# taylorlu/voicepuppet

Measured on AMD Instinct MI355X. Metric: PixReferNet G+D step frames/sec @256x256 bs=32, higher is better.
Workload: dtype bf16; 1 GPU; PixReferNet G+D training step (G + 3xD + VGG16-conv3_3 perceptual + TF-Adam x2), 256x256, ngf=ndf=64, global batch 32 = 32 per GPU; global_batch=32, per_gpu_batch=32, parallelism=dp1

## Files before the change

include/vp_hip.h:

```cpp
#ifndef VP_HIP_H_
#define VP_HIP_H_

#include <stddef.h>
#include <stdint.h>

#ifdef __cplusplus
extern "C" {
#endif

enum vp_status { VP_OK = 0, VP_ERR_ARG = -1, VP_ERR_HIP = -2, VP_ERR_WORKSPACE = -3, VP_ERR_STATE = -4 };
enum vp_dtype { VP_F32 = 0, VP_BF16 = 1 };
enum vp_act { VP_ACT_NONE = 0, VP_ACT_LRELU = 1, VP_ACT_RELU = 2, VP_ACT_TANH = 3, VP_ACT_SIGMOID = 4, VP_ACT_RELU6 = 5, VP_ACT_LEAKY = 6 };

int vp_version(void);
const char* vp_last_error(void);

typedef struct vp_pixrefer_desc {
  int batch;
  int height;
  int ngf, ndf;
  int dtype;
  int training;
  float l1_weight;
  float gan_weight;
  int per_sample_bn;
  int streams;
  int d_backward_fork;
  int d_beside_vgg;
} vp_pixrefer_desc;

size_t vp_pixrefer_desc_size(void);

typedef struct vp_pixrefer vp_pixrefer_t;

size_t vp_pixrefer_param_count(const vp_pixrefer_desc* d, int which);
int vp_pixrefer_param_info(const vp_pixrefer_desc* d, int which, int index, char* name, int name_cap,
                           size_t* offset, int* ndim, int64_t shape[4]);

size_t vp_pixrefer_workspace_bytes(const vp_pixrefer_desc* d);
int vp_pixrefer_validate_plan(const vp_pixrefer_desc* d);

int vp_pixrefer_create(const vp_pixrefer_desc* d, void* workspace, size_t workspace_bytes,
                       float* params_g, float* params_d, const float* params_vgg,
                       float* grads_g, float* grads_d, void* stream, vp_pixrefer_t** out);
void vp_pixrefer_destroy(vp_pixrefer_t* h);

int vp_pixrefer_params_changed(vp_pixrefer_t* h);
int vp_pixrefer_optimizer_stepped(vp_pixrefer_t* h);

int vp_pixrefer_forward(vp_pixrefer_t* h, const float* inputs, const float* fg_inputs,
                        const float* targets, const float* masks, void* stream);

int vp_pixrefer_forward_fg3(vp_pixrefer_t* h, const float* inputs, const float* fg_inputs3, const float* targets, void* stream);

int vp_pixrefer_backward(vp_pixrefer_t* h, void* stream);
int vp_pixrefer_backward_update(vp_pixrefer_t* h, float* m_g, float* v_g, float* m_d, float* v_d, int step_t_g, int step_t_d,
                                float lr, float beta1, float beta2, float eps, void* stream);

int vp_pixrefer_backward_d(vp_pixrefer_t* h, void* stream);
int vp_pixrefer_backward_g(vp_pixrefer_t* h, void* stream);
int vp_pixrefer_backward_d_fork(vp_pixrefer_t* h, void* stream);
int vp_pixrefer_backward_d_join(vp_pixrefer_t* h, void* stream);
void* vp_pixrefer_side_stream(vp_pixrefer_t* h);
int vp_reserve_streams(void);
void* vp_host_stream(void);
int vp_pixrefer_use_streams(vp_pixrefer_t* h, int n);
int vp_pixrefer_set_option(vp_pixrefer_t* h, const char* key, int value);
long long vp_pixrefer_counter(vp_pixrefer_t* h, const char* key);
int vp_pixrefer_fetch(vp_pixrefer_t* h, int what, void* dst, void* stream);
int vp_pixrefer_backward_g_stages(void);
int vp_pixrefer_backward_g_stage(vp_pixrefer_t* h, int stage, void* stream);
int vp_pixrefer_update_bucket(vp_pixrefer_t* h, int which, int bucket, float* m, float* v, int step_t, float lr, float beta1,
                              float beta2, float eps, void* stream);

int vp_pixrefer_tensor(vp_pixrefer_t* h, const char* name, void** ptr, int64_t shape[4], int* dtype);

int vp_profile_enable(int on);
size_t vp_profile_collect(char* json, size_t cap);

int vp_pixrefer_pack_frames(const unsigned char* example_frames, const unsigned char* current_frames, const int* crops,
                            int n, int img_size, float* inputs, float* fg_inputs, float* targets, float* masks, void* stream);

int vp_tune(const char* key, int value);
int vp_pixrefer_phase_ms(vp_pixrefer_t* h, float* ms, int cap);
float vp_pixrefer_mark_ms(vp_pixrefer_t* h, int from, int to);

int vp_grad_pack_bf16(const float* src, void* dst_bf16, size_t n, void* stream);
int vp_grad_unpack_bf16(const void* src_bf16, float* dst, size_t n, float scale, void* stream);

int vp_adam_tf(float* params, const float* grads, float* m, float* v, size_t n, int step_t,
               float lr, float beta1, float beta2, float eps, void* stream);

typedef struct vp_conv_desc {
  int kind;
  int n, h, w;
  int cin, cout;
  int ksize, stride, pad;
  int dtype;
  int in_act;
  int out_act;
} vp_conv_desc;

size_t vp_conv_workspace_bytes(const vp_conv_desc* d);
int vp_conv_fwd(const vp_conv_desc* d, const void* x, const float* in_scale, const float* in_shift,
                const float* w, const float* bias, void* y, void* workspace, void* stream);
int vp_conv_bwd_data(const vp_conv_desc* d, const void* dy, const float* w, void* dx, void* workspace, void* stream);
size_t vp_conv3x3_c64_bwd_data_pooled_workspace_bytes(const vp_conv_desc* d);
int vp_conv3x3_c64_bwd_data_pooled(const vp_conv_desc* d, const void* dy_pool, const unsigned char* code, const float* w, const void* ref,
                                   void* dx, void* workspace, int fused, void* stream);
int vp_conv_bwd_weight(const vp_conv_desc* d, const void* x, const float* in_scale, const float* in_shift,
                       const void* dy, float* dw, void* workspace, void* stream);

size_t vp_bn_workspace_bytes(int pixels, int c, int dtype);
int vp_bn_stats(const void* y, int pixels, int c, int dtype, const float* gamma, const float* beta, float eps,
                float* scale, float* shift, float* mean, float* rstd, void* workspace, void* stream);
int vp_bn_bwd(const void* y, const void* dz, void* dy, int pixels, int c, int dtype, const float* gamma,
              const float* mean, const float* rstd, float* dgamma, float* dbeta, void* workspace, void* stream);

typedef struct vp_logmel_desc {
  int sample_rate, num_mel_bins, win_length, hop_step, fft_length;
  float lower_hz, upper_hz;
  int batch, samples;
} vp_logmel_desc;
typedef struct vp_logmel vp_logmel_t;
size_t vp_logmel_workspace_bytes(const vp_logmel_desc* d);
int vp_logmel_frames(const vp_logmel_desc* d);
int vp_logmel_create(const vp_logmel_desc* d, void* workspace, size_t workspace_bytes, void* stream, vp_logmel_t** out);
void vp_logmel_destroy(vp_logmel_t* h);
int vp_logmel_forward(vp_logmel_t* h, const float* pcm, float* out, void* stream);

typedef struct vp_bfmnet_desc {
  int batch;
  int frames;
  int num_mel_bins;
  int trunk_dtype;
} vp_bfmnet_desc;
typedef struct vp_bfmnet vp_bfmnet_t;
size_t vp_bfmnet_param_count(void);
int vp_bfmnet_param_info(int index, char* name, int name_cap, size_t* offset, int* ndim, int64_t shape[4]);
size_t vp_bfmnet_workspace_bytes(const vp_bfmnet_desc* d);
int vp_bfmnet_create(const vp_bfmnet_desc* d, void* workspace, size_t workspace_bytes, const float* params,
                     void* stream, vp_bfmnet_t** out);
void vp_bfmnet_destroy(vp_bfmnet_t* h);
int vp_bfmnet_params_changed(vp_bfmnet_t* h);
int vp_bfmnet_forward(vp_bfmnet_t* h, const float* ears, const float* mfccs, const int* seq_len, float* out, void* stream);
int vp_bfmnet_set_decoder_dropout(vp_bfmnet_t* h, const float* mask0, const float* mask1);
int vp_bfmnet_tensor(vp_bfmnet_t* h, const char* name, void** ptr, int64_t shape[4]);

typedef struct vp_bfmstream_desc {
  int struct_bytes;
  int max_chunk_frames;
// ... 217 lines not shown
```

voicepuppet_amd/_lib.py:

```python
import ctypes
import os

_HERE = os.path.dirname(os.path.abspath(__file__))
LIB_PATH = os.environ.get("VP_LIB", os.path.join(_HERE, "libvp_hip.so"))

VP_F32, VP_BF16 = 0, 1
ACT_NONE, ACT_LRELU, ACT_RELU, ACT_TANH, ACT_SIGMOID = 0, 1, 2, 3, 4


class PixReferDesc(ctypes.Structure):
  _fields_ = [("batch", ctypes.c_int), ("height", ctypes.c_int), ("ngf", ctypes.c_int), ("ndf", ctypes.c_int),
              ("dtype", ctypes.c_int), ("training", ctypes.c_int), ("l1_weight", ctypes.c_float),
              ("gan_weight", ctypes.c_float), ("per_sample_bn", ctypes.c_int),
              ("streams", ctypes.c_int), ("d_backward_fork", ctypes.c_int), ("d_beside_vgg", ctypes.c_int)]


class ConvDesc(ctypes.Structure):
  _fields_ = [("kind", ctypes.c_int), ("n", ctypes.c_int), ("h", ctypes.c_int), ("w", ctypes.c_int),
              ("cin", ctypes.c_int), ("cout", ctypes.c_int), ("ksize", ctypes.c_int), ("stride", ctypes.c_int),
              ("pad", ctypes.c_int), ("dtype", ctypes.c_int), ("in_act", ctypes.c_int), ("out_act", ctypes.c_int)]


class LogMelDesc(ctypes.Structure):
  _fields_ = [("sample_rate", ctypes.c_int), ("num_mel_bins", ctypes.c_int), ("win_length", ctypes.c_int),
              ("hop_step", ctypes.c_int), ("fft_length", ctypes.c_int), ("lower_hz", ctypes.c_float),
              ("upper_hz", ctypes.c_float), ("batch", ctypes.c_int), ("samples", ctypes.c_int)]


class BfmNetDesc(ctypes.Structure):
  _fields_ = [("batch", ctypes.c_int), ("frames", ctypes.c_int), ("num_mel_bins", ctypes.c_int), ("trunk_dtype", ctypes.c_int)]


class BfmStreamDesc(ctypes.Structure):
  _fields_ = [("struct_bytes", ctypes.c_int), ("max_chunk_frames", ctypes.c_int), ("num_mel_bins", ctypes.c_int),
              ("trunk_dtype", ctypes.c_int), ("sample_rate", ctypes.c_int), ("lower_hz", ctypes.c_float), ("upper_hz", ctypes.c_float)]


class BfmStreamGroupDesc(ctypes.Structure):
  _fields_ = [("struct_bytes", ctypes.c_int), ("slots", ctypes.c_int), ("max_chunk_frames", ctypes.c_int), ("num_mel_bins", ctypes.c_int),
              ("trunk_dtype", ctypes.c_int), ("sample_rate", ctypes.c_int), ("lower_hz", ctypes.c_float), ("upper_hz", ctypes.c_float)]


BFMSTREAM_GROUP_MAX_SLOTS = 128


class PuppetDesc(ctypes.Structure):
  _fields_ = [("struct_bytes", ctypes.c_int), ("slots", ctypes.c_int), ("frame_batch", ctypes.c_int), ("img_size", ctypes.c_int),
              ("face_size", ctypes.c_int)]


PUPPET_MAX_SLOTS = 128


class JpegDesc(ctypes.Structure):
  _fields_ = [("struct_bytes", ctypes.c_uint32), ("max_frames", ctypes.c_int32), ("height", ctypes.c_int32), ("width", ctypes.c_int32),
              ("quality", ctypes.c_int32)]


class PcmInDesc(ctypes.Structure):
  _fields_ = [("struct_bytes", ctypes.c_int), ("slots", ctypes.c_int), ("out_rate", ctypes.c_int), ("max_in_frames", ctypes.c_int),
              ("n_rates", ctypes.c_int), ("rates", ctypes.c_int * 8)]


PCMIN_MAX_SLOTS, PCMIN_MAX_CHANNELS = 128, 8
PCM_S16, PCM_F32 = 0, 1


class BfmModel(ctypes.Structure):
  _fields_ = [("nver", ctypes.c_int), ("ntri", ctypes.c_int), ("meanshape", ctypes.c_void_p), ("idBase", ctypes.c_void_p),
              ("exBase", ctypes.c_void_p), ("meantex", ctypes.c_void_p), ("texBase", ctypes.c_void_p), ("tri", ctypes.c_void_p),
              ("point_buf", ctypes.c_void_p), ("center", ctypes.c_double * 3), ("focal", ctypes.c_double),
              ("image_center", ctypes.c_double), ("sh", ctypes.c_double * 5)]


_P = ctypes.c_void_p
_SIGNATURES = {
    "vp_version": (ctypes.c_int, []),
    "vp_last_error": (ctypes.c_char_p, []),
    "vp_pixrefer_param_count": (ctypes.c_size_t, [ctypes.POINTER(PixReferDesc), ctypes.c_int]),
    "vp_pixrefer_param_info": (ctypes.c_int, [ctypes.POINTER(PixReferDesc), ctypes.c_int, ctypes.c_int, ctypes.c_char_p,
                                              ctypes.c_int, ctypes.POINTER(ctypes.c_size_t), ctypes.POINTER(ctypes.c_int),
                                              ctypes.POINTER(ctypes.c_int64)]),
    "vp_pixrefer_workspace_bytes": (ctypes.c_size_t, [ctypes.POINTER(PixReferDesc)]),
    "vp_pixrefer_validate_plan": (ctypes.c_int, [ctypes.POINTER(PixReferDesc)]),
    "vp_pixrefer_create": (ctypes.c_int, [ctypes.POINTER(PixReferDesc), _P, ctypes.c_size_t, _P, _P, _P, _P, _P, _P,
                                          ctypes.POINTER(_P)]),
    "vp_pixrefer_destroy": (None, [_P]),
    "vp_pixrefer_params_changed": (ctypes.c_int, [_P]),
    "vp_pixrefer_optimizer_stepped": (ctypes.c_int, [_P]),
    "vp_pixrefer_forward": (ctypes.c_int, [_P, _P, _P, _P, _P, _P]),
    "vp_pixrefer_forward_fg3": (ctypes.c_int, [_P, _P, _P, _P, _P]),
    "vp_pixrefer_desc_size": (ctypes.c_size_t, []),
    "vp_pixrefer_backward": (ctypes.c_int, [_P, _P]),
    "vp_pixrefer_backward_update": (ctypes.c_int, [_P, _P, _P, _P, _P, ctypes.c_int, ctypes.c_int, ctypes.c_float, ctypes.c_float,
                                                   ctypes.c_float, ctypes.c_float, _P]),
    "vp_pixrefer_backward_d": (ctypes.c_int, [_P, _P]),
    "vp_pixrefer_backward_g": (ctypes.c_int, [_P, _P]),
    "vp_pixrefer_backward_d_fork": (ctypes.c_int, [_P, _P]),
    "vp_pixrefer_backward_d_join": (ctypes.c_int, [_P, _P]),
    "vp_pixrefer_backward_g_stages": (ctypes.c_int, []),
    "vp_pixrefer_backward_g_stage": (ctypes.c_int, [_P, ctypes.c_int, _P]),
    "vp_pixrefer_side_stream": (ctypes.c_void_p, [_P]),
    "vp_pixrefer_use_streams": (ctypes.c_int, [_P, ctypes.c_int]),
    "vp_pixrefer_set_option": (ctypes.c_int, [_P, ctypes.c_char_p, ctypes.c_int]),
    "vp_pixrefer_fetch": (ctypes.c_int, [_P, ctypes.c_int, _P, _P]),
    "vp_pixrefer_counter": (ctypes.c_longlong, [_P, ctypes.c_char_p]),
    "vp_crc32c": (ctypes.c_uint, [_P, ctypes.c_size_t, ctypes.c_uint]),
    "vp_pixrefer_phase_ms": (ctypes.c_int, [_P, ctypes.POINTER(ctypes.c_float), ctypes.c_int]),
    "vp_grad_pack_bf16": (ctypes.c_int, [_P, _P, ctypes.c_size_t, _P]),
    "vp_grad_unpack_bf16": (ctypes.c_int, [_P, _P, ctypes.c_size_t, ctypes.c_float, _P]),
    "vp_pixrefer_update_bucket": (ctypes.c_int, [_P, ctypes.c_int, ctypes.c_int, _P, _P, ctypes.c_int, ctypes.c_float, ctypes.c_float, ctypes.c_float,
                                                 ctypes.c_float, _P]),
    "vp_resize_paste_workspace_bytes": (ctypes.c_size_t, [ctypes.c_int, ctypes.c_int]),
    "vp_resize_paste_u8": (ctypes.c_int, [_P, ctypes.c_int, ctypes.c_int, ctypes.c_int, ctypes.c_int, ctypes.c_int, ctypes.c_int, _P, ctypes.c_int,
                                          ctypes.c_int, ctypes.c_int, ctypes.c_int, _P, _P]),
    "vp_resize_linear_table": (ctypes.c_int, [ctypes.c_int, ctypes.c_int, ctypes.c_int, _P, _P, _P, _P]),
    "vp_mm_workspace_bytes": (ctypes.c_size_t, [ctypes.c_int, ctypes.c_int, ctypes.c_int]),
    "vp_mm_fwd_f32": (ctypes.c_int, [_P, ctypes.c_int, _P, ctypes.c_int, ctypes.c_int, _P, _P, ctypes.c_int, ctypes.c_int, ctypes.c_int, ctypes.c_int, _P, _P]),
    "vp_mm_bwd_data_f32": (ctypes.c_int, [_P, ctypes.c_int, _P, ctypes.c_int, ctypes.c_int, _P, ctypes.c_int, ctypes.c_int, ctypes.c_int, ctypes.c_int,
                                          ctypes.c_int, _P, _P]),
    "vp_mm_bwd_weight_f32": (ctypes.c_int, [_P, ctypes.c_int, _P, ctypes.c_int, _P, ctypes.c_int, ctypes.c_int, ctypes.c_int, ctypes.c_int, _P, _P]),
    "vp_mm_packed_bytes": (ctypes.c_size_t, [ctypes.c_int, ctypes.c_int, ctypes.c_int, ctypes.c_int]),
    "vp_mm_pack_desc_bytes": (ctypes.c_size_t, []),
    "vp_mm_pack_desc": (ctypes.c_int, [ctypes.c_size_t, ctypes.c_int, ctypes.c_int, ctypes.c_int, ctypes.c_int, ctypes.c_int, ctypes.c_int, ctypes.c_size_t, _P]),
    "vp_mm_pack_table": (ctypes.c_int, [_P, ctypes.c_int, _P, _P, _P]),
    "vp_mm_fwd_f32_packed": (ctypes.c_int, [_P, ctypes.c_int, _P, _P, _P, ctypes.c_int, ctypes.c_int, ctypes.c_int, ctypes.c_int, _P, _P]),
    "vp_mm_bwd_data_f32_packed": (ctypes.c_int, [_P, ctypes.c_int, _P, _P, ctypes.c_int, ctypes.c_int, ctypes.c_int, ctypes.c_int, ctypes.c_int, _P, _P]),
    "vp_pixrefer_mark_ms": (ctypes.c_float, [_P, ctypes.c_int, ctypes.c_int]),
    "vp_profile_enable": (ctypes.c_int, [ctypes.c_int]),
    "vp_tune": (ctypes.c_int, [ctypes.c_char_p, ctypes.c_int]),
    "vp_reserve_streams": (ctypes.c_int, []),
    "vp_host_stream": (ctypes.c_void_p, []),
    "vp_pixrefer_pack_frames": (ctypes.c_int, [_P, _P, _P, ctypes.c_int, ctypes.c_int, _P, _P, _P, _P, _P]),
    "vp_profile_collect": (ctypes.c_size_t, [ctypes.c_char_p, ctypes.c_size_t]),
    "vp_pixrefer_tensor": (ctypes.c_int, [_P, ctypes.c_char_p, ctypes.POINTER(_P), ctypes.POINTER(ctypes.c_int64),
                                          ctypes.POINTER(ctypes.c_int)]),
    "vp_adam_tf": (ctypes.c_int, [_P, _P, _P, _P, ctypes.c_size_t, ctypes.c_int, ctypes.c_float, ctypes.c_float,
                                  ctypes.c_float, ctypes.c_float, _P]),
    "vp_conv_workspace_bytes": (ctypes.c_size_t, [ctypes.POINTER(ConvDesc)]),
    "vp_conv_fwd": (ctypes.c_int, [ctypes.POINTER(ConvDesc), _P, _P, _P, _P, _P, _P, _P, _P]),
    "vp_conv_bwd_data": (ctypes.c_int, [ctypes.POINTER(ConvDesc), _P, _P, _P, _P, _P]),
    "vp_conv_bwd_weight": (ctypes.c_int, [ctypes.POINTER(ConvDesc), _P, _P, _P, _P, _P, _P, _P]),
    "vp_conv3x3_c64_bwd_data_pooled_workspace_bytes": (ctypes.c_size_t, [ctypes.POINTER(ConvDesc)]),
    "vp_conv3x3_c64_bwd_data_pooled": (ctypes.c_int, [ctypes.POINTER(ConvDesc), _P, _P, _P, _P, _P, _P, ctypes.c_int, _P]),
    "vp_bn_workspace_bytes": (ctypes.c_size_t, [ctypes.c_int, ctypes.c_int, ctypes.c_int]),
    "vp_bn_stats": (ctypes.c_int, [_P, ctypes.c_int, ctypes.c_int, ctypes.c_int, _P, _P, ctypes.c_float, _P, _P, _P, _P, _P, _P]),
    "vp_logmel_workspace_bytes": (ctypes.c_size_t, [ctypes.POINTER(LogMelDesc)]),
    "vp_logmel_frames": (ctypes.c_int, [ctypes.POINTER(LogMelDesc)]),
    "vp_logmel_create": (ctypes.c_int, [ctypes.POINTER(LogMelDesc), _P, ctypes.c_size_t, _P, ctypes.POINTER(_P)]),
    "vp_logmel_destroy": (None, [_P]),
    "vp_logmel_forward": (ctypes.c_int, [_P, _P, _P, _P]),
    "vp_bfmnet_param_count": (ctypes.c_size_t, []),
    "vp_bfmnet_param_info": (ctypes.c_int, [ctypes.c_int, ctypes.c_char_p, ctypes.c_int, ctypes.POINTER(ctypes.c_size_t),
                                            ctypes.POINTER(ctypes.c_int), ctypes.POINTER(ctypes.c_int64)]),
    "vp_bfmnet_workspace_bytes": (ctypes.c_size_t, [ctypes.POINTER(BfmNetDesc)]),
    "vp_bfmnet_create": (ctypes.c_int, [ctypes.POINTER(BfmNetDesc), _P, ctypes.c_size_t, _P, _P, ctypes.POINTER(_P)]),
    "vp_bfmnet_destroy": (None, [_P]),
    "vp_bfmnet_params_changed": (ctypes.c_int, [_P]),
    "vp_bfmnet_forward": (ctypes.c_int, [_P, _P, _P, _P, _P, _P]),
    "vp_bfmnet_set_decoder_dropout": (ctypes.c_int, [_P, _P, _P]),
    "vp_bfmnet_tensor": (ctypes.c_int, [_P, ctypes.c_char_p, ctypes.POINTER(_P), ctypes.POINTER(ctypes.c_int64)]),
    "vp_bfmstream_desc_size": (ctypes.c_size_t, []),
    "vp_bfmstream_context": (ctypes.c_int, [ctypes.POINTER(BfmStreamDesc)] + [ctypes.POINTER(ctypes.c_int)] * 5),
    "vp_bfmstream_frames_after": (ctypes.c_longlong, [ctypes.POINTER(BfmStreamDesc), ctypes.c_longlong, ctypes.c_int]),
    "vp_bfmstream_workspace_bytes": (ctypes.c_size_t, [ctypes.POINTER(BfmStreamDesc)]),
    "vp_bfmstream_create": (ctypes.c_int, [ctypes.POINTER(BfmStreamDesc), _P, ctypes.c_size_t, _P, _P, ctypes.POINTER(_P)]),
    "vp_bfmstream_destroy": (None, [_P]),
    "vp_bfmstream_params_changed": (ctypes.c_int, [_P]),
    "vp_bfmstream_reset": (ctypes.c_int, [_P, _P]),
    "vp_bfmstream_ready": (ctypes.c_int, [_P, ctypes.c_longlong]),
    "vp_bfmstream_ready_finish": (ctypes.c_int, [_P]),
    "vp_bfmstream_push": (ctypes.c_int, [_P, _P, ctypes.c_longlong, _P, _P, _P]),
    "vp_bfmstream_finish": (ctypes.c_int, [_P, _P, _P, _P]),
    "vp_bfmstream_tensor": (ctypes.c_int, [_P, ctypes.c_char_p, ctypes.POINTER(_P), ctypes.POINTER(ctypes.c_int64)]),
    "vp_bfmstream_group_desc_size": (ctypes.c_size_t, []),
    "vp_puppet_desc_size": (ctypes.c_size_t, []),
    "vp_puppet_workspace_bytes": (ctypes.c_size_t, [ctypes.POINTER(PuppetDesc)]),
    "vp_puppet_create": (ctypes.c_int, [ctypes.POINTER(PuppetDesc), _P, ctypes.c_size_t, _P, ctypes.POINTER(_P)]),
    "vp_puppet_destroy": (None, [_P]),
    "vp_puppet_attach": (ctypes.c_int, [_P, ctypes.c_int, _P, _P, _P, ctypes.c_int, ctypes.c_int, ctypes.c_int, _P]),
    "vp_puppet_set_backgrounds": (ctypes.c_int, [_P, _P, ctypes.c_int]),
    "vp_puppet_splice": (ctypes.c_int, [_P, _P, ctypes.c_int, _P, ctypes.c_int, _P, _P]),
    "vp_puppet_condition": (ctypes.c_int, [_P, _P, ctypes.c_int, _P, ctypes.c_int, _P, _P, _P, _P]),
    "vp_puppet_tensor": (ctypes.c_int, [_P, ctypes.c_char_p, ctypes.POINTER(_P), ctypes.POINTER(ctypes.c_int64)]),
    "vp_puppet_slot_info": (ctypes.c_int, [_P, ctypes.c_int, ctypes.POINTER(ctypes.c_int)]),
    "vp_jpeg_desc_size": (ctypes.c_size_t, []),
    "vp_jpeg_workspace_bytes": (ctypes.c_size_t, [ctypes.POINTER(JpegDesc)]),
    "vp_jpeg_frame_capacity": (ctypes.c_size_t, [ctypes.POINTER(JpegDesc)]),
    "vp_jpeg_create": (ctypes.c_int, [ctypes.POINTER(JpegDesc), _P, ctypes.c_size_t, _P, ctypes.POINTER(_P)]),
# ... 134 lines not shown
```

voicepuppet_amd/csrc/conv_ops.h:

```cpp
#pragma once
#include <stdlib.h>
#include <string.h>

#include "launch.h"

namespace vp {

struct ConvGeomX : ConvGeom {
  int CoutT;
};

inline ConvGeomX make_geom(int kind, int ks, int stride, int pad, int N, int Hin, int Win, int Cin, int Cin_real, int Cout) {
  ConvGeomX g;
  g.kind = kind; g.ks = ks; g.stride = stride; g.pad = pad;
  g.N = N; g.Hin = Hin; g.Win = Win;
  if (kind == 0) { g.Hout = (Hin + 2 * pad - ks) / stride + 1; g.Wout = (Win + 2 * pad - ks) / stride + 1; }
  else { g.Hout = 2 * Hin; g.Wout = 2 * Win; }
  g.Cin = Cin; g.Cin_real = Cin_real; g.Cout = Cout;
  g.CoutT = Cout < 8 ? 8 : Cout;
  return g;
}

inline int kc_elems(int is_bf16) { return is_bf16 ? 32 : 16; }

// ... 10 lines not shown
    if (rows % 128 == 0) return 0;
    if (rows % 64 == 0) return 1;
    if (rows <= 16) return 2;
    return rows > 64 ? 0 : 1;
  }
  if (rows <= 64) return 5;
  return P > 16 ? 3 : 4;
}

constexpr int IGEMM_SPLITK_TARGET_DEFAULT = 64;
inline int& igemm_splitk_target_knob() { static int v = IGEMM_SPLITK_TARGET_DEFAULT; return v; }
inline int pick_igemm_splitk(int blocks, int nchunk) {
  const int target = igemm_splitk_target_knob();
  const int cap = plan_misc_knob(1);
  const int minchunk = plan_misc_knob(2);
  if (blocks >= 256 || blocks >= target) return 1;
  int s = (target + blocks - 1) / blocks;
  if (s > nchunk / minchunk) s = nchunk / minchunk;
  if (s > cap) s = cap;
  return s < 1 ? 1 : s;
}

inline void set_single_src(PixSrc& x, const void* p, int C, const float* a, const float* b, int act, int group_n) {
  x.ptr[0] = p; x.ptr[1] = nullptr; x.C[0] = C; x.C[1] = 0;
  x.aff_a[0] = a; x.aff_b[0] = b; x.aff_a[1] = nullptr; x.aff_b[1] = nullptr;
  x.act = act; x.group_n = group_n > 0 ? group_n : (1 << 30);
}

struct LaunchForm {
  bool bias = false, ref = false, xa_lrelu = false, xa_relu = false, x_affine = false;
  bool stats = false;
  int x_act = 0, ref_act = 0;
};

struct IgemmPlan {
  IgemmArgs a;
  int cfg;
  LaunchForm form;
  PackDesc pack;
  size_t pack_elems;
  size_t partial_bytes;
};

struct IgemmPin { int cfg, splitk; };

inline void finish_igemm(IgemmPlan& p, int rows, int is_bf16, const IgemmPin* pin = nullptr) {
  IgemmArgs& a = p.a;
  const int P = a.N * a.Hg * a.Wg;
  a.Kpad = round_up(a.ntaps * a.Cin, kc_elems(is_bf16));
  p.cfg = pick_igemm_cfg(rows, P, a.Kpad);
  if (!is_bf16 && a.ntaps == 1 && p.cfg == 0) {
    const long long b128 = (long long)((P + 127) / 128) * (rows / 128), b64 = 2 * b128;
    if (((b64 + 255) / 256) * 64 < ((b128 + 255) / 256) * 128) p.cfg = 1;
  }
  if (pin) p.cfg = pin->cfg;
  int bc, bp;
  igemm_tile(p.cfg, &bc, &bp);
  a.CoutPad = round_up(rows, bc);
  if (a.ntaps == 1) { a.log2Cin = 30; a.cin_mask = 0x3fffffff; }
  else { a.log2Cin = ilog2(a.Cin); a.cin_mask = a.Cin - 1; }
  const int blocks = ((P + bp - 1) / bp) * (a.CoutPad / bc) * a.nclass;
  a.splitk = pin ? pin->splitk : pick_igemm_splitk(blocks, a.Kpad / kc_elems(is_bf16));
  p.partial_bytes = a.splitk > 1 ? (size_t)a.nclass * a.splitk * P * a.CoutPad * sizeof(float) : 0;
  {
    const bool tc4 = p.cfg == 0 || p.cfg == 1 || p.cfg == 6 || p.cfg == 7 || p.cfg == 8 || p.cfg == 9;
    a.rowperm = (tc4 && rows % 64 == 0) ? 1 : 0;
    p.pack.perm = a.rowperm;
  }
  a.wp_rows = round_up(rows, 128);
  p.pack.rows_pad = a.wp_rows;
  p.pack.Kpad = a.Kpad;
  p.pack.kc = kc_elems(is_bf16);
  p.pack_elems = (size_t)a.nclass * a.wp_rows * a.Kpad;
}

inline int& patch_tiles_knob() { static int v = 7; return v; }
inline int& patch_small_knob() { static int v = 3; return v; }
inline int& patch_longk_knob() { static int v = 1; return v; }
inline int& patch3_knob() { static int v = 1; return v; }
inline int& wgrad_big_knob() { static int v = 1; return v; }
inline int& patch4_knob() { static int v = 1; return v; }
inline int& c64_knob() { static int v = 1; return v; }
inline int& pool_bwd_fused_knob() { static int v = 1; return v; }
inline int& cout1_knob() { static int v = 256; return v; }
inline int& wgrad1_rows_knob() { static int v = 512; return v; }
inline int& dc64_knob() { static int v = 1; return v; }
inline int& s2c64_knob() { static int v = 512; return v; }
inline int& s2c64_pair_knob() { static int v = 1; return v; }
constexpr int PATCH_MIN_BLOCKS_DEFAULT = 192;
inline int& patch_minblk_knob() { static int v = PATCH_MIN_BLOCKS_DEFAULT; return v; }

inline void patch_tile_hw(int bp, int* th, int* tw) { *th = bp == 128 ? 8 : 16; *tw = bp == 512 ? 32 : 16; }
inline int patch_tile_pixels(int bc) {
  const int k = patch_small_knob();
  if (bc == 256) return (k & 2) ? 128 : 256;
  return (k & 1) ? 256 : 512;
}

inline int patch_tile_rows(int rows, int on) {
  if ((on & 1) && rows % 256 == 0) return 256;
  if ((on & 2) && rows % 128 == 0) return 128;
  if ((on & 4) && rows % 64 == 0) return 64;
  return 0;
}

inline bool plan_patch_eligible(const IgemmPlan& p, int rows, int is_bf16, bool single_src, bool any_grid = false) {
  const int on = patch_tiles_knob();
  const int minblk = any_grid ? 0 : patch_minblk_knob();
  const IgemmArgs& a = p.a;
  const int kc = kc_elems(is_bf16);
  if (!on || !single_src || a.nclass != 1 || a.sh != 1 || a.sw != 1 || a.os != 1 || a.ntaps < 9 || a.Cin % kc || a.Cin < kc) return false;
  if (rows % 64 || a.Cout % 8 || a.ldY % 8 || a.Hg < 16 || a.Wg < 16 || a.Hof != a.Hg || a.Wof != a.Wg) return false;
  const bool p4 = patch4_knob() && is_bf16 && a.ntaps == 16 && rows % 128 == 0;
  if (!p4 && patch_longk_knob() && rows >= 512 && rows % 256 == 0 && a.ntaps * a.Cin >= 4096 && (long long)a.N * a.Hg * a.Wg >= 256 * 256) return false;
  const int bc = p4 ? 128 : patch_tile_rows(rows, on);
  if (!bc) return false;
  int th, tw;
  patch_tile_hw(p4 ? 256 : patch_tile_pixels(bc), &th, &tw);
  const long long blocks = (long long)a.N * ((a.Hg + th - 1) / th) * ((a.Wg + tw - 1) / tw) * (rows / bc);
  const long long p4min = (long long)a.ntaps * a.Cin >= 8192 ? 256 : 512;
  if (p4 && !any_grid && patch_minblk_knob() > 1) {
    if (blocks < p4min) return false;
  } else if (blocks < minblk) return false;
  if ((size_t)a.N * a.Hin * a.Win * a.Cin * (is_bf16 ? 2 : 4) >= 0x70000000ull) return false;
  int ks = 0;
  while (ks * ks < a.ntaps) ++ks;
  if (ks * ks != a.ntaps) return false;
  const int sh = a.taps[0].dh[ks] - a.taps[0].dh[0], sw = a.taps[0].dw[1] - a.taps[0].dw[0];
  if ((sh != 1 && sh != -1) || (sw != 1 && sw != -1)) return false;
  for (int t = 0; t < a.ntaps; ++t)
    if (a.taps[0].dh[t] != a.taps[0].dh[0] + (t / ks) * sh || a.taps[0].dw[t] != a.taps[0].dw[0] + (t % ks) * sw) return false;
  return true;
}
inline void plan_make_patch(IgemmPlan& p, int rows, int is_bf16) {
  IgemmArgs& a = p.a;
  const bool p4 = patch4_knob() && is_bf16 && a.ntaps == 16 && rows % 128 == 0;
  const int bc = p4 ? 128 : patch_tile_rows(rows, patch_tiles_knob());
  int ks = 0;
  while (ks * ks < a.ntaps) ++ks;
  a.kern = CK_PATCH; a.p_kw = ks;
  a.p_dhf = a.taps[0].dh[0]; a.p_dwf = a.taps[0].dw[0];
  a.p_dhs = a.taps[0].dh[ks] - a.taps[0].dh[0]; a.p_dws = a.taps[0].dw[1] - a.taps[0].dw[0];
  const int bp = p4 ? 256 : patch_tile_pixels(bc);
  p.cfg = bc == 256 ? (bp == 128 ? 15 : 10) : (bc == 128 ? (bp == 256 ? 13 : 11) : (bp == 256 ? 14 : 12));
  a.CoutPad = round_up(rows, bc);
  a.splitk = 1;
  p.partial_bytes = 0;
  a.rowperm = 1;
  p.pack.perm = 1;
  p.pack.kswap = 1;
}

inline int& patch_xcd_knob() { static int v = 0; return v; }
inline int& patch2_knob() { static int v = 1; return v; }
inline bool plan_patch2_eligible(const IgemmPlan& p, int rows, int is_bf16, int c0, int c1) {
  const IgemmArgs& a = p.a;
  const int kc = kc_elems(is_bf16);
  if (!patch2_knob() || a.nclass != 4 || a.ntaps != 4 || a.os != 2 || a.sh != 1 || a.sw != 1) return false;
  if (c0 + c1 != a.Cin || c0 % (2 * kc) || c1 % (2 * kc) || c0 < 2 * kc) return false;
  if (rows % 64 || rows > 128 || a.Cout % 8 || a.ldY % 8 || a.Hg < 16 || a.Wg < 16 || a.Hof != 2 * a.Hg || a.Wof != 2 * a.Wg) return false;
  const long long blocks = (long long)a.N * ((a.Hg + 15) / 16) * ((a.Wg + 15) / 16) * 4;
  if (blocks < patch_minblk_knob()) return false;
  const size_t cmax = c0 > c1 ? c0 : c1;
  if ((size_t)a.N * a.Hin * a.Win * cmax * (is_bf16 ? 2 : 4) >= 0x70000000ull) return false;
  for (int cls = 0; cls < 4; ++cls)
    for (int t = 0; t < 4; ++t)
// ... 281 lines not shown
```

voicepuppet_amd/csrc/launch.h:

```cpp
#pragma once
#include <hip/hip_runtime.h>

#include "conv_args.h"
#include "pointwise_args.h"

namespace vp {

hipError_t launch_igemm(const IgemmArgs& a, int is_bf16, int cfg, hipStream_t st);
void igemm_tile(int cfg, int* bc, int* bp);
hipError_t launch_igemm_patch(const IgemmArgs& a, int is_bf16, int bc, int bp, hipStream_t st);
bool patch3_eligible(const IgemmArgs& a, int is_bf16);
hipError_t launch_igemm_patch3(const IgemmArgs& a, int is_bf16, int bc, int bp, hipStream_t st);
bool patch4_eligible(const IgemmArgs& a, int is_bf16);
hipError_t launch_igemm_patch4(const IgemmArgs& a, hipStream_t st);
bool conv_cin8_eligible(const IgemmArgs& a, int is_bf16);
bool conv_cout8_eligible(const IgemmArgs& a, int is_bf16);
bool conv_dcout8_eligible(const IgemmArgs& a, int is_bf16);
bool conv_cout4_eligible(const IgemmArgs& a, int is_bf16);
bool conv_kernel_ok(const IgemmArgs& a, int is_bf16);
const char* conv_kernel_name(int kern);
bool conv_c64_eligible(const IgemmArgs& a, int is_bf16);
hipError_t launch_conv_c64(const IgemmArgs& a, hipStream_t st);
bool conv_dc64_eligible(const IgemmArgs& a, int is_bf16);
hipError_t launch_conv_dc64(const IgemmArgs& a, hipStream_t st);
int conv_dc64_grid(const IgemmArgs& a);
bool conv_dc256_eligible(const IgemmArgs& a, int is_bf16);
int conv_dc256_grid(const IgemmArgs& a);
hipError_t launch_conv_dc256(const IgemmArgs& a, hipStream_t st);
bool conv_s2c64_eligible(const IgemmArgs& a, int is_bf16);
int conv_s2c64_grid(const IgemmArgs& a);
int conv_s2c64_tiles_per_image(const IgemmArgs& a);
hipError_t launch_conv_s2c64(const IgemmArgs& a, hipStream_t st);
bool conv_cout1_bwd_eligible(const Cout1Args& a);
hipError_t launch_conv_cout1_bwd(const Cout1Args& a, hipStream_t st);
bool conv_cout1_wgrad_eligible(const Cout1Args& a);
hipError_t launch_conv_cout1_wgrad(const Cout1Args& a, hipStream_t st);
hipError_t launch_cout1_wgrad_prof(const Cout1Args& a, hipStream_t st);
hipError_t launch_cout1_bwd_prof(const Cout1Args& a, hipStream_t st);
hipError_t launch_igemm_patch2(const IgemmArgs& a, int is_bf16, int bc, int bp, hipStream_t st);
hipError_t launch_igemm_smallp(const IgemmArgs& a, int is_bf16, hipStream_t st);
struct SmallPArgs;
hipError_t launch_smallp(const SmallPArgs& s, int is_bf16, hipStream_t st);
hipError_t launch_smallp_fused(const SmallPArgs& s, int is_bf16, hipStream_t st);
hipError_t launch_wgrad(const WgradArgs& a, int is_bf16, int cfg, hipStream_t st);
bool wgrad_mm_eligible(const WgradArgs& a, int cfg);
hipError_t launch_wgrad_mm(const WgradArgs& a, int cfg, hipStream_t st);
hipError_t launch_wgrad_tr(const WgradArgs& a, hipStream_t st, const char** variant = nullptr, int* tile_cols = nullptr);
void wgrad_tile(int cfg, int* bm, int* bn);

void profile_enable(int on);
void profile_tag(const char* tag);
size_t profile_collect(char* out, size_t cap);

hipError_t launch_pack_weights(const PackDesc* d_descs, int ndesc, const float* master, void* packed, int is_bf16, hipStream_t st);
hipError_t launch_pack_weights_one(const PackDesc& d, const float* master, void* packed, int is_bf16, hipStream_t st);
int bn_nchunk(int Pg, int C, int G, int is_bf16);
hipError_t launch_bn_stats(const BnArgs& a, int is_bf16, hipStream_t st);
hipError_t launch_bn_finalize(const BnArgs& a, hipStream_t st);
bool bn_small(const BnArgs& a);
hipError_t launch_bn_small_fwd(const BnArgs& a, void* out_lrelu, void* out_relu, int is_bf16, hipStream_t st);
hipError_t launch_bn_small_bwd(const BnArgs& a, int is_bf16, hipStream_t st);
hipError_t launch_bn_bwd(const BnArgs& a, int is_bf16, hipStream_t st);
hipError_t launch_bn_bwd_tail(const BnArgs& a, int is_bf16, hipStream_t st);
hipError_t launch_colsum(const BnArgs& a, int creal, float* out, int accumulate, int is_bf16, hipStream_t st);
hipError_t launch_colsum_tail(const BnArgs& a, int creal, float* out, int accumulate, hipStream_t st);
hipError_t launch_act_apply(const void* y, const float* sc, const float* sh, int C, int Pg, size_t npix,
                            void* out_lrelu, void* out_relu, int is_bf16, hipStream_t st);
hipError_t launch_tap_gather(const TapArgs& a, hipStream_t st);
hipError_t launch_tap_spread(const TapArgs& a, int is_bf16, hipStream_t st);
hipError_t launch_frame_pack(const FramePackArgs& a, hipStream_t st);
hipError_t launch_pack_inputs(const PackInputsArgs& a, int is_bf16, hipStream_t st);
int composite_nblocks(int N, int HW);
hipError_t launch_composite_fwd(const CompositeArgs& a, int is_bf16, hipStream_t st);
hipError_t launch_composite_bwd(const CompositeArgs& a, int is_bf16, hipStream_t st);
hipError_t launch_gan_loss(const GanLossArgs& a, int is_bf16, hipStream_t st);
int perceptual_nblocks(size_t half, int is_bf16);
hipError_t launch_perceptual(const PerceptualArgs& a, int is_bf16, hipStream_t st);
hipError_t launch_loss_final(const LossFinalArgs& a, hipStream_t st);
hipError_t launch_maxpool_fwd(const void* x, void* y, int B, int H, int W, int C, int is_bf16, hipStream_t st);
hipError_t launch_maxpool_bwd(const void* x, const void* dy, void* dx, int B, int H, int W, int C, int is_bf16, hipStream_t st);
hipError_t launch_maxpool_bwd_code(const void* code, const void* dy, void* dx, int B, int H, int W, int C, int is_bf16, hipStream_t st);
hipError_t launch_relu_bwd(const void* y, void* d, size_t n, int is_bf16, hipStream_t st);
hipError_t launch_adam(const AdamArgs& a, hipStream_t st);
hipError_t launch_fetch(const FetchArgs& a, hipStream_t st);
hipError_t launch_grad_pack_bf16(const float* src, void* dst, size_t n, hipStream_t st);
hipError_t launch_grad_unpack_bf16(const void* src, float* dst, size_t n, float scale, hipStream_t st);

struct ConvGeom {
  int kind;
  int ks, stride, pad;
  int N, Hin, Win, Hout, Wout;
  int Cin, Cin_real;
  int Cout;
};

inline int ilog2(int v) { int l = 0; while ((1 << l) < v) ++l; return l; }
inline int round_up(int v, int m) { return (v + m - 1) / m * m; }

}
```

voicepuppet_amd/csrc/ops_api.hip:

```cpp
#include <string.h>

#include <string>

#include "conv_ops.h"
#include "errors.h"
#include "audio_args.h"
#include "launch.h"
#include "vp_common.h"

using namespace vp;

namespace {

bool conv_desc_ok(const vp_conv_desc* d) {
  if (!d || d->n < 1 || d->h < 1 || d->w < 1) return false;
  if (d->cin < 8 || (d->cin & (d->cin - 1))) return false;
  if (d->kind == 1 && (d->ksize != 4 || d->stride != 2 || d->pad != 1)) return false;
  if (d->kind != 0 && d->kind != 1) return false;
  if (d->ksize < 1 || d->ksize > 4 || d->stride < 1 || d->stride > 2) return false;
  if (d->kind == 0 && d->stride == 2 && (d->ksize != 4 || d->pad != 1 || (d->h & 1) || (d->w & 1))) return false;
  return d->dtype == VP_F32 || d->dtype == VP_BF16;
}

ConvGeomX geom_of(const vp_conv_desc* d) {
  return make_geom(d->kind, d->ksize, d->stride, d->pad, d->n, d->h, d->w, d->cin, d->cin, d->cout);
}

size_t align256(size_t v) { return (v + 255) & ~(size_t)255; }

const void* zero_page(char* ws, size_t used, hipStream_t st) {
  char* z = ws + align256(used);
  (void)hipMemsetAsync(z, 0, 256, st);
  return z;
}

}

extern "C" {

int vp_pixrefer_pack_frames(const unsigned char* example_frames, const unsigned char* current_frames, const int* crops,
                            int n, int img_size, float* inputs, float* fg_inputs, float* targets, float* masks, void* stream) {
  if (!example_frames || !current_frames || !crops || !inputs || !fg_inputs || !targets || !masks || n < 1 || img_size < 2) {
    set_err("vp_pixrefer_pack_frames: bad argument");
    return VP_ERR_ARG;
  }
  FramePackArgs a;
  a.ex = example_frames; a.cur = current_frames; a.crops = crops;
  a.inputs = inputs; a.fg_inputs = fg_inputs; a.targets = targets; a.masks = masks;
  a.N = n; a.S = img_size;
  VP_HIP_CHECK(launch_frame_pack(a, (hipStream_t)stream));
  return VP_OK;
}

extern "C" void vp_phase_marks_enable(int on);

int vp_tune(const char* key, int value) {
  if (!key) return VP_ERR_ARG;
  const std::string k(key);
  if (k == "patch_tiles") { patch_tiles_knob() = value; return VP_OK; }
  if (k == "patch_min_blocks") { patch_minblk_knob() = value < 0 ? PATCH_MIN_BLOCKS_DEFAULT : value; return VP_OK; }
  if (k == "patch_small_tiles") { patch_small_knob() = value; return VP_OK; }
  if (k == "patch_long_k_on_256") { patch_longk_knob() = value; return VP_OK; }
  if (k == "wgrad_tr") { wgrad_tr_knob() = value; return VP_OK; }
  if (k == "patch3") { patch3_knob() = value; return VP_OK; }
  if (k == "c64") { c64_knob() = value; return VP_OK; }
  if (k == "dc64") { dc64_knob() = value; return VP_OK; }
  if (k == "pool_bwd_fused") { pool_bwd_fused_knob() = value < 0 || value > 4 ? 1 : value; return VP_OK; }
  if (k == "cout1_wgrad_rows" && value > 0) { wgrad1_rows_knob() = value; return VP_OK; }
  if (k == "cout1_bwd") { cout1_knob() = value < 0 ? 256 : value; return VP_OK; }
  if (k == "s2c64") { s2c64_knob() = value; return VP_OK; }
  if (k == "wgrad_big") { wgrad_big_knob() = value; return VP_OK; }
  if (k == "patch4") { patch4_knob() = value; return VP_OK; }
  if (k == "s2c64_pair") { s2c64_pair_knob() = value; return VP_OK; }
  if (k == "bfm_dwproj") { bfm_dwproj_knob() = value; return VP_OK; }
  if (k == "patch2") { patch2_knob() = value; return VP_OK; }
  if (k == "patch_xcd") { patch_xcd_knob() = value; return VP_OK; }
  if (k == "smallp_max_pixels") { smallp_knob() = value; return VP_OK; }
  if (k == "igemm_splitk_target") { igemm_splitk_target_knob() = value < 0 ? IGEMM_SPLITK_TARGET_DEFAULT : value; return VP_OK; }
  if (k == "wgrad_fixed_x10") { wgrad_cost_knob(0) = value; return VP_OK; }
  if (k == "wgrad_slab_tile_x1000") { wgrad_cost_knob(2) = value < 0 ? 150 : value; return VP_OK; }
  if (k == "wgrad_slab_x100") { wgrad_cost_knob(1) = value; return VP_OK; }
  if (k == "smallp_split_target") { plan_misc_knob(0) = value; return VP_OK; }
  if (k == "igemm_splitk_cap") { plan_misc_knob(1) = value; return VP_OK; }
  if (k == "igemm_splitk_minchunk") { plan_misc_knob(2) = value; return VP_OK; }
  if (k == "wgrad_resident_blocks") { plan_misc_knob(3) = value; return VP_OK; }
  if (k == "igemm_small_grid") { igemm_small_grid_knob() = value; return VP_OK; }
  if (k == "thin_blocks_cout8" && value > 0) { thin_blocks_knob(0) = value; return VP_OK; }
  if (k == "thin_blocks_dcout8" && value > 0) { thin_blocks_knob(1) = value; return VP_OK; }
  if (k == "thin_blocks_cout4" && value > 0) { thin_blocks_knob(2) = value; return VP_OK; }
  if (k == "thin_blocks_cin8" && value > 0) { thin_blocks_knob(3) = value; return VP_OK; }
  if (k == "phase_marks") { vp_phase_marks_enable(value); return VP_OK; }
  set_err("vp_tune: unknown key %s", key);
  return VP_ERR_ARG;
}

static unsigned* smallp_counter_page(char* ws, size_t used, const IgemmArgs& a, hipStream_t st) {
  unsigned* c = (unsigned*)(ws + align256(used) + 256);
  (void)hipMemsetAsync(c, 0, (size_t)smallp_counters(a) * sizeof(unsigned), st);
  return c;
}

size_t vp_conv_workspace_bytes(const vp_conv_desc* d) {
  if (!conv_desc_ok(d)) return 0;
  const int bf = d->dtype == VP_BF16, es = bf ? 2 : 4;
  const ConvGeomX g = geom_of(d);
  size_t best = 0;
  {
    IgemmPlan p = plan_fwd(g, 0, bf);
    best = align256(p.pack_elems * es) + p.partial_bytes;
    plan_kernel(p, g.Cout, bf, d->cin, 0, FAM_SMALLP, LaunchForm{});
    if (p.a.kern == CK_SMALLP) {
      const size_t b = align256(p.pack_elems * es) + align256(p.partial_bytes) + 512 + (size_t)smallp_counters(p.a) * sizeof(unsigned);
      if (b > best) best = b;
    }
  }
  if ((d->cout & (d->cout - 1)) == 0 && d->cout >= 8) {
    IgemmPlan p = plan_bwd_data(g, 0, 0, d->cin, d->cin, d->cin, bf);
    size_t b = align256(p.pack_elems * es) + p.partial_bytes;
    if (b > best) best = b;
    plan_kernel(p, d->cin, bf, d->cout, 0, FAM_SMALLP, LaunchForm{});
    if (p.a.kern == CK_SMALLP) {
      b = align256(p.pack_elems * es) + align256(p.partial_bytes) + 512 + (size_t)smallp_counters(p.a) * sizeof(unsigned);
      if (b > best) best = b;
    }
    for (int plain = 0; plain < 2; ++plain) {
      WgradPlan w = plan_wgrad(g, bf, plain != 0);
      if (w.partial_bytes + 512 > best) best = w.partial_bytes + 512;
    }
  }
  return best + 1024;
}

int vp_conv_fwd(const vp_conv_desc* d, const void* x, const float* in_scale, const float* in_shift,
                const float* w, const float* bias, void* y, void* workspace, void* stream) {
  if (!conv_desc_ok(d) || !x || !w || !y || !workspace) { set_err("vp_conv_fwd: bad argument"); return VP_ERR_ARG; }
  const int bf = d->dtype == VP_BF16, es = bf ? 2 : 4;
  hipStream_t st = (hipStream_t)stream;
  const ConvGeomX g = geom_of(d);
  IgemmPlan p = plan_fwd(g, 0, bf);
  p.a.out_act = d->out_act;
  LaunchForm f;
  f.bias = bias != nullptr; f.x_affine = in_scale != nullptr; f.x_act = d->in_act;
  const bool plain = d->in_act == ACT_NONE && !in_scale;
  plan_kernel(p, g.Cout, bf, d->cin, 0, plain ? (FAM_SMALLP | FAM_PATCH | FAM_PATCH2 | (d->out_act == ACT_NONE ? FAM_S2C64 : 0)) : 0, f);
  char* ws = (char*)workspace;
  VP_HIP_CHECK(launch_pack_weights_one(p.pack, w, ws, bf, st));
  IgemmArgs a = p.a;
  set_single_src(a.x, x, d->cin, in_scale, in_shift, d->in_act, 0);
  a.Wp = ws;
  a.partial = (float*)(ws + align256(p.pack_elems * es));
// ... 276 lines not shown
```

voicepuppet_amd/csrc/plan_pixrefer.hip:

```cpp
#include <math.h>
#include <stdio.h>
#include <string.h>

#include <mutex>
#include <string>
#include <utility>
#include <vector>

#include "conv_ops.h"
#include "errors.h"
#include "launch.h"
#include "smallp_args.h"
#include "vp_common.h"

namespace vp {

thread_local char g_err[512] = "";
void set_err(const char* fmt, ...) {
  va_list ap;
  va_start(ap, fmt);
  vsnprintf(g_err, sizeof(g_err), fmt, ap);
  va_end(ap);
}

struct Arena {
  char* base;
  size_t off, cap;
  std::vector<std::pair<size_t, size_t>>* track = nullptr;
  void* alloc(size_t bytes) {
    off = (off + 255) & ~(size_t)255;
    void* p = base ? base + off : nullptr;
    if (track) track->push_back({off, bytes});
    off += bytes;
    return p;
  }
};

struct BnBuf {
  float *a, *b, *mu, *rstd, *c1, *c2, *c1g, *c2g;
  double *pb, *pbg;
};

struct Tens {
  std::string name;
  void* y = nullptr;
  void* dz = nullptr;
  int N = 0, H = 0, W = 0, C = 0;
  bool is_f32 = false;
  bool has_bn = false;
  bool is_input = false;
  bool dz_written = false;
  void* dz2 = nullptr;
  bool dz2_written = false;
  void* xa[3] = {nullptr, nullptr, nullptr};
  bool need_act[3] = {false, false, false};
  BnBuf bn{};
  int producer = -1;
  int n_bwd_consumers = 0;
  int dz_writes = 0;
  bool bn_bwd_done = false;
  bool hi = false;
  void* dz32 = nullptr;
  double* cs_part = nullptr;
  int cs_chunks = 0;
  int pb_cap = 0, pbg_cap = 0;
  int bst_chunks = 0, bst_chunks_g = 0;
  size_t elems() const { return (size_t)N * H * W * C; }
};

struct Layer {
  std::string scope;
  ConvGeomX g;
  int src[2] = {-1, -1};
  int nsrc = 1;
  int in_act = ACT_NONE;
  int out_act = ACT_NONE;
  int out = -1;
  bool has_bn = false;
  size_t w_off = 0, b_off = 0, gamma_off = 0, beta_off = 0;
  size_t pk_fwd = 0, pk_bwd[2] = {0, 0}, pk_bwd_alt[2] = {0, 0};
  bool need_bwd[2] = {false, false};
  IgemmPlan fwd, bwd[2], bwd_alt[2];
  IgemmPlan bwd_pair;
  size_t pk_bwd_pair = 0;
  bool has_pair = false;
  IgemmPlan fwd_half;
  size_t pk_fwd_half = 0;
  bool has_fwd_half = false;
  WgradPlan wg;
  size_t desc0 = 0, desc1 = 0;
  bool tapgemm = false;
  bool fwd_stats = false;
  float* tap_S = nullptr;
  void* tap_dyS = nullptr;
  unsigned* sp_cnt_fwd = nullptr;
  unsigned* sp_cnt_bwd[2] = {nullptr, nullptr};
  unsigned* sp_cnt_pair = nullptr;
};

struct ParamInfo { std::string name; size_t off; int ndim; int64_t shape[4]; };

struct Net {
  std::vector<Tens> t;
  std::vector<Layer> l;
  std::vector<ParamInfo> manifest;
  size_t nparams = 0;
  int batch = 0, groups = 1;
  float* params = nullptr;
  float* grads = nullptr;
  char* packed = nullptr;
  size_t packed_elems = 0;
  std::vector<PackDesc> descs;
  PackDesc* d_descs = nullptr;
  unsigned* sp_cnt = nullptr;
  size_t sp_cnt_n = 0;
};

}

using namespace vp;

struct vp_pixrefer {
  vp_pixrefer_desc d;
  int bf16, es;
  Net G, D, V;
  void *gin, *gfg, *din, *vin;
  float *y4, *o4, *outputs, *outputs_fg, *logits, *predict, *losses;
  void *dl_d, *dl_g, *d_din, *d_vin, *dy4, *df3;
  void *vpool1, *vpool2, *d_vpool1, *d_vpool2;
  unsigned char* vpool_code[2];
  bool pool_codes_written;
  bool pool_fuse_ok[2];
  bool pool_bwd_fused;
  bool pool_dz_stale[2];
  double *comp_partial, *perc_partial, *bn_partial;
  char* scratch;
  char* scratch2;
  double* bn_partial2;
  char* scratch3;
  double* bn_partial3;
  char* scratch4;
  double* bn_partial4;
  hipStream_t side, branch;
  hipStream_t branch2;
  hipEvent_t ev_b2join;
  bool use_b2;
  hipEvent_t ev_fork, ev_join, ev_bfork, ev_bjoin;
  hipEvent_t ev_upd_b, ev_upd_m;
  bool overlap, forked;
  int bst_count;
  int bst_on;
  int vgg_fork_layer;
  bool store_first_raw;
  bool ov_on;
  int dfork_point;
  bool dsplit_on;
  hipEvent_t mark[64];
  int nmark;
  bool marks_made;
  int dfork_pending;
  void* zeros;
  size_t scratch_bytes;
  int n_comp, n_perc;
  struct { bool active, d_done; float *m_g, *v_g, *m_d, *v_d; float lr_t_g, lr_t_d, beta1, beta2, eps; } upd;
  int upd_mask;
  bool params_dirty;
  bool vgg_dirty;
  const float *in_targets, *in_masks;
};

namespace vp {

static int add_tensor(Net& n, const std::string& name, int N, int H, int W, int C, bool has_bn, bool is_input) {
  Tens t;
  t.name = name; t.N = N; t.H = H; t.W = W; t.C = C; t.has_bn = has_bn; t.is_input = is_input;
  n.t.push_back(t);
  return (int)n.t.size() - 1;
}

static void add_param(Net& n, const std::string& name, std::initializer_list<int64_t> shape, size_t* off_out) {
  ParamInfo p;
  p.name = name; p.off = n.nparams; p.ndim = (int)shape.size();
  size_t cnt = 1;
  int i = 0;
  for (auto s : shape) { p.shape[i++] = s; cnt *= (size_t)s; }
  for (; i < 4; ++i) p.shape[i] = 1;
  *off_out = n.nparams;
  n.nparams += cnt;
  n.manifest.push_back(p);
}

static int add_layer(Net& n, const std::string& prefix, const std::string& scope, int kind, int ks, int stride, int pad,
                     std::initializer_list<int> srcs, int cin_real, int cout, bool has_bn, int in_act, int out_act,
                     const char* wname, const char* bname) {
  Layer L;
  L.scope = scope;
// ... 176 lines not shown
            take(L.bwd_alt[s]);
            L.pk_bwd_alt[s] = L.bwd_alt[s].pack.dst_off;
          } else {
            L.bwd_alt[s].pack.dst_off = L.pk_bwd[s];
            if (L.bwd_alt[s].partial_bytes > *scratch_max) *scratch_max = L.bwd_alt[s].partial_bytes;
          }
        }
      }
      row0 += rows;
    }
    {
      const int s0 = conv_staging(L.bwd[0].a.kern);
      if (L.nsrc == 2 && n.groups == 1 && alt_batch == 0 && L.need_bwd[0] && L.need_bwd[1] && c0 == c1 && !n.t[L.src[0]].is_input &&
          !n.t[L.src[1]].is_input && s0 == conv_staging(L.bwd[1].a.kern) && (s0 == CK_IGEMM || s0 == CK_SMALLP) &&
          L.g.Cin_real == c0 + c1 && c0 % 32 == 0) {
        L.bwd_pair = plan_bwd_data(L.g, L.w_off, 0, c0 + c1, c0 + c1, c0, bf16);
        L.bwd_pair.a.split_c = c0;
        LaunchForm f;
        f.ref = true; f.ref_act = L.in_act;
        const unsigned fams = s0 == CK_SMALLP ? FAM_SMALLP : (s2c64_pair_knob() && L.in_act == ACT_RELU ? FAM_S2C64 : 0);
        plan_kernel(L.bwd_pair, c0 + c1, bf16, L.g.CoutT, 0, fams, f);
        if (s0 != CK_SMALLP || L.bwd_pair.a.kern == CK_SMALLP) {
          take(L.bwd_pair);
          L.pk_bwd_pair = L.bwd_pair.pack.dst_off;
          L.has_pair = true;
        }
      }
    }
    if (want_wgrad) {
      if (L.tapgemm) {
        ConvGeomX gw = make_geom(0, 1, 1, 0, L.g.N, L.g.Hin, L.g.Win, 16, 16, L.g.Cin);
        L.wg = plan_wgrad(gw, bf16);
      } else {
        L.wg = plan_wgrad(L.g, bf16);
      }
      if (L.wg.partial_bytes > *scratch_max) *scratch_max = L.wg.partial_bytes;
    }
  }
  n.packed_elems = pk;
  {
    for (Tens& t : n.t) t.hi = bf16 && t.has_bn && n.groups == 1 && alt_batch == 0 && t.producer >= 0 && n.l[t.producer].fwd.a.kern == CK_SMALLP;
    if (training)
      for (Layer& L : n.l)
        for (int s = 0; s < L.nsrc; ++s)
          if (L.need_bwd[s] && L.bwd[s].a.kern != CK_SMALLP) n.t[L.src[s]].hi = false;
    for (Layer& L : n.l)
      for (int s = 0; s < L.nsrc; ++s)
        if (L.in_act == ACT_NONE) n.t[L.src[s]].hi = false;
  }
  for (Tens& t : n.t) t.pb_cap = t.pbg_cap = 0;
  if (training)
    for (Layer& L : n.l) {
      auto cap = [&](Tens& t, const IgemmPlan& p, int batch, int groups, int& c) {
        if (!t.has_bn || t.hi) return;
        const int k = epi_stat_chunks(p, batch, groups);
        if (k > 0 && k <= BST_MAX_CHUNKS && k > c) c = k;
      };
      for (int s = 0; s < L.nsrc; ++s) {
        if (!L.need_bwd[s]) continue;
        Tens& ts = n.t[L.src[s]];
        cap(ts, L.bwd[s], n.batch, n.groups, ts.pb_cap);
        if (alt_batch > 0) cap(ts, L.bwd_alt[s], alt_batch, 1, ts.pbg_cap);
        if (L.has_pair) cap(ts, L.bwd_pair, n.batch, n.groups, ts.pb_cap);
        if (L.tapgemm && bf16 && ts.has_bn && !ts.hi && L.g.ks == 4 && L.g.stride == 1 && L.g.Cin == 512) {
          if (ts.pb_cap < 256) ts.pb_cap = 256;
          if (alt_batch > 0 && ts.pbg_cap < 256) ts.pbg_cap = 256;
        }
      }
    }
  for (size_t i = 0; i < n.l.size(); ++i) n.l[i].desc1 = i + 1 < n.l.size() ? n.l[i + 1].desc0 : n.descs.size();
  for (Tens& t : n.t) t.n_bwd_consumers = 0;
  n.sp_cnt_n = 0;
  for (Layer& L : n.l) {
    if (L.fwd.a.kern == CK_SMALLP) n.sp_cnt_n += smallp_counters(L.fwd.a);
    for (int s = 0; s < L.nsrc && training; ++s) {
      if (!L.need_bwd[s]) continue;
      n.t[L.src[s]].n_bwd_consumers++;
      if (L.bwd[s].a.kern == CK_SMALLP) n.sp_cnt_n += smallp_counters(L.bwd[s].a);
    }
    if (training && L.has_pair && L.bwd_pair.a.kern == CK_SMALLP) n.sp_cnt_n += smallp_counters(L.bwd_pair.a);
  }
}

static void carve_net(Net& n, Arena& ar, int es, bool training) {
  for (Tens& t : n.t) {
    if (t.name == "decoder_1" || t.name == "layer_5") {
      continue;
    }
    if (!t.is_input) t.y = ar.alloc(t.elems() * (t.hi ? sizeof(float) : (size_t)es));
    for (int k = 1; k < 3; ++k) if (t.need_act[k]) t.xa[k] = ar.alloc(t.elems() * es);
    if (t.has_bn) {
      const size_t gc = (size_t)n.groups * t.C * sizeof(float);
      t.bn.a = (float*)ar.alloc(gc); t.bn.b = (float*)ar.alloc(gc);
      t.bn.mu = (float*)ar.alloc(gc); t.bn.rstd = (float*)ar.alloc(gc);
      t.bn.c1 = (float*)ar.alloc(gc); t.bn.c2 = (float*)ar.alloc(gc);
      t.bn.c1g = (float*)ar.alloc(gc); t.bn.c2g = (float*)ar.alloc(gc);
      t.bn.pb = (training && t.pb_cap) ? (double*)ar.alloc((size_t)n.groups * t.pb_cap * 2 * t.C * sizeof(double)) : nullptr;
      t.bn.pbg = (training && t.pbg_cap) ? (double*)ar.alloc((size_t)t.pbg_cap * 2 * t.C * sizeof(double)) : nullptr;
    }
  }
  for (Layer& L : n.l) {
    if (!L.tapgemm) continue;
    const size_t q = (size_t)L.g.N * L.g.Hin * L.g.Win * 16;
    L.tap_S = (float*)ar.alloc(q * sizeof(float));
    L.tap_dyS = ar.alloc(q * es);
  }
  n.packed = (char*)ar.alloc(n.packed_elems * es);
  n.d_descs = (PackDesc*)ar.alloc(n.descs.size() * sizeof(PackDesc));
  n.sp_cnt = (unsigned*)ar.alloc((n.sp_cnt_n + 1) * sizeof(unsigned));
  {
    unsigned* c = n.sp_cnt;
    for (Layer& L : n.l) {
      if (L.fwd.a.kern == CK_SMALLP) { L.sp_cnt_fwd = c; c += c ? smallp_counters(L.fwd.a) : 0; }
      for (int s = 0; s < L.nsrc && training; ++s)
        if (L.need_bwd[s] && L.bwd[s].a.kern == CK_SMALLP) { L.sp_cnt_bwd[s] = c; c += c ? smallp_counters(L.bwd[s].a) : 0; }
      if (training && L.has_pair && L.bwd_pair.a.kern == CK_SMALLP) { L.sp_cnt_pair = c; c += c ? smallp_counters(L.bwd_pair.a) : 0; }
    }
  }
}

static size_t carve_all(vp_pixrefer* h, char* base, size_t cap, std::vector<std::pair<size_t, size_t>>* track = nullptr) {
  Arena ar{base, 0, cap};
  ar.track = track;
  const vp_pixrefer_desc& d = h->d;
  const int N = d.batch, H = d.height, es = h->es;
  const size_t px = (size_t)N * H * H;
  h->gin = ar.alloc(px * 8 * es);
  h->gfg = ar.alloc(px * 8 * es);
  h->y4 = (float*)ar.alloc(px * 4 * sizeof(float));
  h->o4 = (float*)ar.alloc(px * 4 * sizeof(float));
  h->outputs = (float*)ar.alloc(px * 3 * sizeof(float));
  h->outputs_fg = (float*)ar.alloc(px * 3 * sizeof(float));
  h->losses = (float*)ar.alloc(8 * sizeof(float));
  h->G.t[0].y = h->gin; h->G.t[1].y = h->gfg;
  carve_net(h->G, ar, es, d.training);
  if (d.training) {
    const int hd = H / 8 - 2;
    const size_t M = (size_t)N * hd * hd;
    h->din = ar.alloc(3 * px * 8 * es);
    h->vin = ar.alloc(2 * px * 8 * es);
    h->logits = (float*)ar.alloc(3 * M * sizeof(float));
    h->predict = (float*)ar.alloc(2 * M * sizeof(float));
    h->dl_d = ar.alloc(3 * M * 8 * es);
    h->dl_g = ar.alloc(M * 8 * es);
    h->d_din = ar.alloc(px * 8 * es);
    h->d_vin = ar.alloc(px * 8 * es);
    h->dy4 = ar.alloc(px * 8 * es);
    h->D.t[0].y = h->din; h->V.t[0].y = h->vin;
    carve_net(h->D, ar, es, true);
    carve_net(h->V, ar, es, true);
    for (Tens& t : h->G.t) if (!t.is_input && t.name != "decoder_1") { t.dz = ar.alloc(t.elems() * es); if (t.hi) t.dz32 = ar.alloc(t.elems() * sizeof(float)); }
    for (Tens& t : h->D.t) if (!t.is_input && t.name != "layer_5") { t.dz = ar.alloc(t.elems() * es); t.dz2 = ar.alloc(t.elems() / 3 * es); }
    for (Net* n : {&h->G, &h->D})
      for (Tens& t : n->t) if (h->bf16 && !t.is_input && !t.has_bn && t.C == 64) t.cs_part = (double*)ar.alloc((size_t)512 * 2 * 64 * sizeof(double));
    for (Tens& t : h->V.t) if (!t.is_input) t.dz = ar.alloc(t.elems() / 2 * es);
    for (const Tens& t : h->V.t) {
      if (t.name == "pool1") h->vpool_code[0] = (unsigned char*)ar.alloc(t.elems() / 2);
      if (t.name == "pool2") h->vpool_code[1] = (unsigned char*)ar.alloc(t.elems() / 2);
    }
    h->n_comp = composite_nblocks(N, H * H);
    h->n_perc = perceptual_nblocks((size_t)N * (H / 4) * (H / 4) * 256, h->bf16);
    h->comp_partial = (double*)ar.alloc((size_t)h->n_comp * 2 * sizeof(double));
    h->perc_partial = (double*)ar.alloc((size_t)h->n_perc * sizeof(double));
  }
  h->zeros = ar.alloc(256);
  h->bn_partial = (double*)ar.alloc((size_t)1024 * 2 * 512 * sizeof(double));
  h->scratch = (char*)ar.alloc(h->scratch_bytes);
  if (d.training) {
    h->bn_partial2 = (double*)ar.alloc((size_t)1024 * 2 * 512 * sizeof(double));
    h->scratch2 = (char*)ar.alloc(h->scratch_bytes);
    h->bn_partial3 = (double*)ar.alloc((size_t)1024 * 2 * 512 * sizeof(double));
    h->scratch3 = (char*)ar.alloc(h->scratch_bytes);
    h->bn_partial4 = (double*)ar.alloc((size_t)1024 * 2 * 512 * sizeof(double));
    h->scratch4 = (char*)ar.alloc(h->scratch_bytes);
  }
  return ar.off + 256;
}

static IgemmArgs pool_fused_view(const IgemmPlan& p) {
  static unsigned char set[16] = {};
  IgemmArgs v = launch_view(p, p.form);
  v.pool_code = set;
  v.pool_src = 1;
  return v;
}

static void init_handle(vp_pixrefer* h, const vp_pixrefer_desc* d) {
  h->d = *d;
  h->bf16 = d->dtype == VP_BF16;
  h->es = h->bf16 ? 2 : 4;
  build_generator(h->G, d->batch, d->height, d->ngf, (!d->training && d->per_sample_bn) ? d->batch : 1);
  size_t smax = 0;
  plan_net(h->G, h->bf16, d->training, d->training, 0, &smax);
  if (d->training) {
    build_discriminator(h->D, d->batch, d->height, d->ndf);
    plan_net(h->D, h->bf16, true, true, d->batch, &smax);
    build_vgg(h->V, d->batch, d->height);
    for (Layer& L : h->V.l) L.g.N = 2 * d->batch;
    plan_net(h->V, h->bf16, true, false, d->batch, &smax, true);
    for (const Layer& L : h->V.l) {
      if (L.scope != "conv1/conv1_2" && L.scope != "conv2/conv2_2") continue;
      const int k = L.scope == "conv2/conv2_2", knob = pool_bwd_fused_knob();
      const IgemmArgs& ba = L.bwd_alt[0].a;
      const bool big = !k || (long long)ba.N * (ba.Hg / 4) * (ba.Wg / 16) >= 4096;
      h->pool_fuse_ok[k] = ((knob == 1 && big) || knob == 2 + k || knob == 4) && h->bf16 && conv_kernel_ok(pool_fused_view(L.bwd_alt[0]), h->bf16);
    }
  }
  h->scratch_bytes = smax + 256;
  h->params_dirty = true;
  h->vgg_dirty = true;
}

static bool valid_desc(const vp_pixrefer_desc* d) {
  if (!d) { set_err("pixrefer descriptor: null"); return false; }
  if (d->batch < 1 || d->height < 256 || d->height % 256 != 0) { set_err("pixrefer descriptor: batch %d / height %d (height must be a multiple of 256)", d->batch, d->height); return false; }
  if (d->ngf < 8 || (d->ngf & (d->ngf - 1)) || d->ndf < 8 || (d->ndf & (d->ndf - 1))) { set_err("pixrefer descriptor: ngf %d / ndf %d must be powers of two >= 8", d->ngf, d->ndf); return false; }
  if (d->ngf > 64 || d->ndf > 64) { set_err("pixrefer descriptor: ngf %d / ndf %d > 64 exceed the batch-norm workspace (512 channels)", d->ngf, d->ndf); return false; }
  if (!d->training && d->per_sample_bn && d->batch > 1024) { set_err("pixrefer descriptor: per-sample batch-norm supports at most 1024 frames per call (got %d)", d->batch); return false; }
  if (d->dtype != VP_F32 && d->dtype != VP_BF16) { set_err("pixrefer descriptor: dtype %d", d->dtype); return false; }
  if ((d->streams != 0 && d->streams != 1 && d->streams != 3 && d->streams != 4) || d->d_backward_fork < 0 || d->d_backward_fork > 3 || d->d_beside_vgg < 0 ||
      d->d_beside_vgg > 2) {
    set_err("pixrefer descriptor: schedule fields streams %d / d_backward_fork %d / d_beside_vgg %d", d->streams, d->d_backward_fork, d->d_beside_vgg);
    return false;
  }
  return true;
}

static void fill_src(const Net& n, const Layer& L, PixSrc& x, int group_n, int sample0, int group0, int es) {
  for (int s = 0; s < 2; ++s) {
    x.ptr[s] = nullptr; x.C[s] = 0; x.aff_a[s] = nullptr; x.aff_b[s] = nullptr;
  }
  for (int s = 0; s < L.nsrc; ++s) {
    const Tens& t = n.t[L.src[s]];
    const void* base = (L.in_act != ACT_NONE) ? t.xa[L.in_act] : t.y;
    x.ptr[s] = (const char*)base + (size_t)sample0 * t.H * t.W * t.C * es;
    x.C[s] = t.C;
  }
  x.act = ACT_NONE;
  x.group_n = group_n;
  (void)group0;
}

static int run_pack(vp_pixrefer* h, Net& n, hipStream_t st) {
  if (n.descs.empty()) return VP_OK;
  VP_HIP_CHECK(launch_pack_weights(n.d_descs, (int)n.descs.size(), n.params, n.packed, h->bf16, st));
  return VP_OK;
}

static char* scratch_of(vp_pixrefer* h, int ss) { return ss == 3 ? h->scratch4 : ss == 2 ? h->scratch3 : ss == 1 ? h->scratch2 : h->scratch; }
static double* bnp_of(vp_pixrefer* h, int ss) { return ss == 3 ? h->bn_partial4 : ss == 2 ? h->bn_partial3 : ss == 1 ? h->bn_partial2 : h->bn_partial; }

static int run_bn_stats(vp_pixrefer* h, Net& n, Layer& L, int fused_chunks, hipStream_t st, int ss = 0) {
  Tens& t = n.t[L.out];
  BnArgs b;
  memset(&b, 0, sizeof(b));
  b.y = t.y; b.C = t.C; b.G = n.groups; b.Pg = (n.batch / n.groups) * t.H * t.W;
  b.nchunk = bn_nchunk(b.Pg, b.C, b.G, h->bf16);
  b.partial = bnp_of(h, ss);
  b.gamma = n.params + L.gamma_off; b.beta = n.params + L.beta_off;
  b.aff_a = t.bn.a; b.aff_b = t.bn.b; b.mu = t.bn.mu; b.rstd = t.bn.rstd;
  b.eps = 1e-5f;
  if (fused_chunks > 0) { b.nchunk = fused_chunks; VP_HIP_CHECK(launch_bn_finalize(b, st)); return VP_OK; }
  if (bn_small(b)) {
    VP_HIP_CHECK(launch_bn_small_fwd(b, t.xa[ACT_LRELU], t.xa[ACT_RELU], h->bf16, st));
    return 1;
  }
  VP_HIP_CHECK(launch_bn_stats(b, h->bf16, st));
  return VP_OK;
}

static bool plan_can_pool(const IgemmPlan& p) {
  if (conv_staging(p.a.kern) != CK_PATCH || (p.a.Hg & 1) || (p.a.Wg & 1)) return false;
  int bc, bp;
  igemm_tile(p.cfg, &bc, &bp);
  int th, tw;
  patch_tile_hw(bp, &th, &tw);
  return tw == 16 && th % 2 == 0;
}

// ... 418 lines not shown
  if (!valid_desc(d)) return 0;
  vp_pixrefer tmp{};
  Net* n = manifest_net(d, which, &tmp);
  return n ? n->nparams : 0;
}

int vp_pixrefer_param_info(const vp_pixrefer_desc* d, int which, int index, char* name, int name_cap,
                           size_t* offset, int* ndim, int64_t shape[4]) {
  if (!valid_desc(d)) return VP_ERR_ARG;
  vp_pixrefer tmp{};
  Net* n = manifest_net(d, which, &tmp);
  if (!n || index < 0 || index >= (int)n->manifest.size()) return VP_ERR_ARG;
  const ParamInfo& p = n->manifest[index];
  if (name && name_cap > 0) { strncpy(name, p.name.c_str(), name_cap - 1); name[name_cap - 1] = 0; }
  if (offset) *offset = p.off;
  if (ndim) *ndim = p.ndim;
  if (shape) for (int i = 0; i < 4; ++i) shape[i] = p.shape[i];
  return VP_OK;
}

size_t vp_pixrefer_workspace_bytes(const vp_pixrefer_desc* d) {
  if (!valid_desc(d)) return 0;
  vp_pixrefer* h = new vp_pixrefer{};
  init_handle(h, d);
  const size_t n = carve_all(h, nullptr, 0);
  delete h;
  return n;
}

int vp_pixrefer_validate_plan(const vp_pixrefer_desc* d) {
  if (!valid_desc(d)) return VP_ERR_ARG;
  vp_pixrefer* h = new vp_pixrefer{};
  init_handle(h, d);
  const size_t need = carve_all(h, nullptr, 0);
  std::vector<std::pair<size_t, size_t>> regs;
  char* const base = reinterpret_cast<char*>((uintptr_t)1 << 40);
  carve_all(h, base, need, &regs);
  int rc = VP_OK;
  auto fail = [&](const char* fmt, auto... args) { if (rc == VP_OK) { set_err(fmt, args...); rc = VP_ERR_STATE; } };
  size_t prev_end = 0;
  for (size_t i = 0; i < regs.size(); ++i) {
    if (regs[i].first % 256) fail("region %zu at %zu: not 256-byte aligned", i, regs[i].first);
    if (regs[i].first < prev_end) fail("region %zu at %zu overlaps the previous one (ends %zu)", i, regs[i].first, prev_end);
    prev_end = regs[i].first + regs[i].second;
  }
  if (prev_end + 256 > need + 256 || prev_end > need) fail("carved %zu bytes of a %zu-byte workspace", prev_end, need);
  auto region_of = [&](const void* p, size_t bytes, const char* what) {
    if (!p) { fail("%s: null", what); return; }
    const size_t off = (size_t)((const char*)p - base);
    for (const auto& r : regs)
      if (off >= r.first && off + bytes <= r.first + r.second) return;
    fail("%s: [%zu, +%zu) is not inside a carved region", what, off, bytes);
  };
  const int es = h->es;
  for (Net* n : {&h->G, &h->D, &h->V}) {
    if (n->t.empty()) continue;
    for (const Tens& t : n->t) {
      const std::string nm = t.name;
      if (t.name == "decoder_1" || t.name == "layer_5") continue;
      region_of(t.y, t.elems() * (t.hi ? 4 : es), (nm + ".y").c_str());
      for (int k = 1; k < 3; ++k) if (t.need_act[k]) region_of(t.xa[k], t.elems() * es, (nm + ".xa").c_str());
      if (t.has_bn) {
        const size_t gc = (size_t)n->groups * t.C * sizeof(float);
        for (const float* p : {t.bn.a, t.bn.b, t.bn.mu, t.bn.rstd, t.bn.c1, t.bn.c2, t.bn.c1g, t.bn.c2g}) region_of(p, gc, (nm + ".bn").c_str());
        if (d->training && t.pb_cap) region_of(t.bn.pb, (size_t)n->groups * t.pb_cap * 2 * t.C * sizeof(double), (nm + ".bn.pb").c_str());
        if (d->training && t.pbg_cap) region_of(t.bn.pbg, (size_t)t.pbg_cap * 2 * t.C * sizeof(double), (nm + ".bn.pbg").c_str());
        if ((size_t)n->groups * t.C > (size_t)1024 * 512) fail("%s: %d groups x %d channels exceed the batch-norm partial rows", nm.c_str(), n->groups, t.C);
      }
      if (t.cs_part) region_of(t.cs_part, (size_t)512 * 2 * 64 * sizeof(double), (nm + ".cs_part").c_str());
      if (d->training && !t.is_input) {
        const size_t div = n == &h->V ? 2 : 1;
        region_of(t.dz, t.elems() / div * es, (nm + ".dz").c_str());
        if (t.hi) region_of(t.dz32, t.elems() * 4, (nm + ".dz32").c_str());
        if (n == &h->D) region_of(t.dz2, t.elems() / 3 * es, (nm + ".dz2").c_str());
      }
    }
    region_of(n->packed, n->packed_elems * es, "packed weights");
    region_of(n->d_descs, n->descs.size() * sizeof(PackDesc), "pack descriptors");
    for (const PackDesc& p : n->descs) {
      const size_t pe = (size_t)p.nclass * p.Kpad * p.rows_pad;
      if (p.dst_off + pe > n->packed_elems) fail("pack block [%zu, +%zu) outside the %zu-element packed arena", p.dst_off, pe, n->packed_elems);
      if (p.src_off >= n->nparams) fail("pack source %zu outside the %zu-float parameter arena", p.src_off, n->nparams);
    }
    size_t pend = 0;
    for (const ParamInfo& p : n->manifest) {
      size_t cnt = 1;
      for (int i = 0; i < 4; ++i) cnt *= (size_t)p.shape[i];
      if (p.off != pend) fail("parameter %s at %zu: arena not contiguous (expected %zu)", p.name.c_str(), p.off, pend);
      pend = p.off + cnt;
    }
    if (pend != n->nparams) fail("parameter manifest covers %zu of %zu floats", pend, n->nparams);
    for (const Layer& L : n->l) {
      auto plan_ok = [&](const IgemmPlan& p, const char* what) {
        if (p.partial_bytes > h->scratch_bytes) fail("%s %s: split-K slab %zu > scratch %zu", L.scope.c_str(), what, p.partial_bytes, h->scratch_bytes);
        if (p.a.splitk < 1 || p.a.CoutPad < p.a.Cout) fail("%s %s: splitk %d CoutPad %d", L.scope.c_str(), what, p.a.splitk, p.a.CoutPad);
        if (!conv_kernel_ok(launch_view(p, p.form), h->bf16))
          fail("%s %s: the launch is outside the preconditions of its kernel %s", L.scope.c_str(), what, conv_kernel_name(p.a.kern));
      };
      plan_ok(L.fwd, "fwd");
      if (L.has_fwd_half) plan_ok(L.fwd_half, "fwd_half");
      if (d->training && L.has_pair) plan_ok(L.bwd_pair, "bwd_pair");
      if (d->training)
        for (int s2 = 0; s2 < L.nsrc; ++s2) if (L.need_bwd[s2]) { plan_ok(L.bwd[s2], "bwd"); if (n == &h->D || n == &h->V) plan_ok(L.bwd_alt[s2], "bwd_alt"); }
      if (d->training && n != &h->V && L.wg.partial_bytes > h->scratch_bytes) fail("%s wgrad: slab %zu > scratch %zu", L.scope.c_str(), L.wg.partial_bytes, h->scratch_bytes);
      if (L.tapgemm) { region_of(L.tap_S, (size_t)L.g.N * L.g.Hin * L.g.Win * 16 * 4, "tap_S"); region_of(L.tap_dyS, (size_t)L.g.N * L.g.Hin * L.g.Win * 16 * es, "tap_dyS"); }
    }
  }
  const size_t px = (size_t)d->batch * d->height * d->height;
  region_of(h->gin, px * 8 * es, "gin"); region_of(h->gfg, px * 8 * es, "gfg");
  region_of(h->y4, px * 4 * 4, "y4"); region_of(h->o4, px * 4 * 4, "o4");
  region_of(h->outputs, px * 3 * 4, "outputs"); region_of(h->outputs_fg, px * 3 * 4, "outputs_fg");
  region_of(h->scratch, h->scratch_bytes, "scratch"); region_of(h->bn_partial, (size_t)1024 * 2 * 512 * 8, "bn_partial");
  if (d->training) {
    const int hd = d->height / 8 - 2;
    const size_t M = (size_t)d->batch * hd * hd;
    region_of(h->din, 3 * px * 8 * es, "din"); region_of(h->vin, 2 * px * 8 * es, "vin");
    region_of(h->logits, 3 * M * 4, "logits"); region_of(h->predict, 2 * M * 4, "predict");
    region_of(h->dl_d, 3 * M * 8 * es, "dl_d"); region_of(h->dl_g, M * 8 * es, "dl_g");
    region_of(h->d_din, px * 8 * es, "d_din"); region_of(h->d_vin, px * 8 * es, "d_vin"); region_of(h->dy4, px * 8 * es, "dy4");
    for (const Tens& t : h->V.t) {
      if (t.name == "pool1") region_of(h->vpool_code[0], t.elems() / 2, "pool1 codes");
      if (t.name == "pool2") region_of(h->vpool_code[1], t.elems() / 2, "pool2 codes");
    }
    for (const Layer& L : h->V.l) {
      const int k = L.scope == "conv2/conv2_2";
      if ((L.scope != "conv1/conv1_2" && !k) || !h->pool_fuse_ok[k]) continue;
      const Tens& tp = h->V.t[L.out + 1];
      if (tp.name != (k ? "pool2" : "pool1") || tp.H * 2 != h->V.t[L.out].H || tp.C != h->V.t[L.out].C) fail("%s: the tensor behind it is not its 2x2 pool", L.scope.c_str());
      if (L.bwd_alt[0].a.kern != CK_C64 || !conv_kernel_ok(pool_fused_view(L.bwd_alt[0]), h->bf16)) fail("%s bwd_alt: no pooled-source form of kernel %s", L.scope.c_str(), conv_kernel_name(L.bwd_alt[0].a.kern));
      region_of(tp.dz, tp.elems() / 2 * es, (tp.name + ".dz (pooled-source read)").c_str());
      region_of(h->vpool_code[k], tp.elems() / 2, (tp.name + " codes (pooled-source read)").c_str());
    }
    region_of(h->scratch2, h->scratch_bytes, "scratch2"); region_of(h->scratch3, h->scratch_bytes, "scratch3");
    region_of(h->scratch4, h->scratch_bytes, "scratch4"); region_of(h->bn_partial4, (size_t)1024 * 2 * 512 * 8, "bn_partial4");
    region_of(h->bn_partial2, (size_t)1024 * 2 * 512 * 8, "bn_partial2"); region_of(h->bn_partial3, (size_t)1024 * 2 * 512 * 8, "bn_partial3");
  }
  delete h;
  return rc;
}

struct StreamPool {
  int dev = -1;
  hipStream_t side = nullptr, branch = nullptr, branch2 = nullptr;
};
static StreamPool g_pool;
static std::mutex g_pool_mu;

static int pool_streams(bool want_b2, hipStream_t* side, hipStream_t* branch, hipStream_t* branch2) {
  std::lock_guard<std::mutex> lk(g_pool_mu);
  int dev = 0;
  VP_HIP_CHECK(hipGetDevice(&dev));
  if (g_pool.dev >= 0 && g_pool.dev != dev) { set_err("the step executor's streams were created on device %d, this plan is on device %d (one device per process)", g_pool.dev, dev); return VP_ERR_STATE; }
  if (!g_pool.side) {
    int prio_lo = 0, prio_hi = 0;
    (void)hipDeviceGetStreamPriorityRange(&prio_lo, &prio_hi);
    VP_HIP_CHECK(hipStreamCreateWithPriority(&g_pool.side, hipStreamNonBlocking, prio_lo));
    VP_HIP_CHECK(hipStreamCreateWithFlags(&g_pool.branch, hipStreamNonBlocking));
    g_pool.dev = dev;
  }
  if (want_b2 && !g_pool.branch2) VP_HIP_CHECK(hipStreamCreateWithFlags(&g_pool.branch2, hipStreamNonBlocking));
  if (side) *side = g_pool.side;
  if (branch) *branch = g_pool.branch;
  if (branch2) *branch2 = g_pool.branch2;
  return VP_OK;
}

int vp_reserve_streams(void) { return pool_streams(true, nullptr, nullptr, nullptr); }

void* vp_host_stream(void) {
  hipStream_t b2 = nullptr;
  if (pool_streams(true, nullptr, nullptr, &b2)) return nullptr;
  return (void*)b2;
}

int vp_pixrefer_create(const vp_pixrefer_desc* d, void* workspace, size_t workspace_bytes,
                       float* params_g, float* params_d, const float* params_vgg,
                       float* grads_g, float* grads_d, void* stream, vp_pixrefer_t** out) {
  if (!valid_desc(d) || !workspace || !params_g || !out) { set_err("vp_pixrefer_create: bad argument"); return VP_ERR_ARG; }
  if (d->training && (!params_d || !params_vgg || !grads_g || !grads_d)) { set_err("training needs D/VGG params and grad arenas"); return VP_ERR_ARG; }
  vp_pixrefer* h = new vp_pixrefer{};
  init_handle(h, d);
  const size_t need = carve_all(h, nullptr, 0);
  if (workspace_bytes < need) { set_err("workspace too small: %zu < %zu", workspace_bytes, need); delete h; return VP_ERR_WORKSPACE; }
  carve_all(h, (char*)workspace, workspace_bytes);
  h->G.params = params_g; h->G.grads = grads_g;
  h->D.params = params_d; h->D.grads = grads_d;
  h->V.params = const_cast<float*>(params_vgg);
  for (Tens& t : h->G.t) if (t.name == "decoder_1") { t.y = h->y4; t.dz = h->dy4; }
  hipStream_t st = (hipStream_t)stream;
  VP_HIP_CHECK(hipMemsetAsync(h->zeros, 0, 256, st));
  if (d->training) for (Tens& t : h->D.t) if (t.name == "layer_5") { t.y = h->logits; t.dz = h->dl_d; }
  for (Net* n : {&h->G, &h->D, &h->V}) {
    if (n->descs.empty()) continue;
    VP_HIP_CHECK(hipMemcpyAsync(n->d_descs, n->descs.data(), n->descs.size() * sizeof(PackDesc), hipMemcpyHostToDevice, st));
    VP_HIP_CHECK(hipMemsetAsync(n->sp_cnt, 0, (n->sp_cnt_n + 1) * sizeof(unsigned), st));
  }
  VP_HIP_CHECK(hipStreamSynchronize(st));
  h->overlap = false; h->forked = false;
  h->bst_on = 1; h->vgg_fork_layer = 3;
  h->ov_on = true; h->store_first_raw = false; h->dfork_point = d->d_backward_fork ? d->d_backward_fork - 1 : 2; h->dsplit_on = d->d_beside_vgg != 1;
  if (d->training && d->streams != 1) {
    { const int rc = pool_streams(false, &h->side, &h->branch, &h->branch2); if (rc) { delete h; return rc; } }
    VP_HIP_CHECK(hipEventCreateWithFlags(&h->ev_fork, hipEventDisableTiming));
    VP_HIP_CHECK(hipEventCreateWithFlags(&h->ev_join, hipEventDisableTiming));
    h->use_b2 = d->streams != 3;
    VP_HIP_CHECK(hipEventCreateWithFlags(&h->ev_b2join, hipEventDisableTiming));
    VP_HIP_CHECK(hipEventCreateWithFlags(&h->ev_bfork, hipEventDisableTiming));
    VP_HIP_CHECK(hipEventCreateWithFlags(&h->ev_bjoin, hipEventDisableTiming));
    VP_HIP_CHECK(hipEventCreateWithFlags(&h->ev_upd_b, hipEventDisableTiming));
    VP_HIP_CHECK(hipEventCreateWithFlags(&h->ev_upd_m, hipEventDisableTiming));
    h->overlap = true;
  }
  *out = h;
  return VP_OK;
}

void vp_pixrefer_destroy(vp_pixrefer_t* h) {
  if (!h) return;
  if (h->marks_made) for (int i = 0; i < 64; ++i) (void)hipEventDestroy(h->mark[i]);
  if (h->overlap) {
    (void)hipStreamSynchronize(h->side);
    (void)hipEventDestroy(h->ev_fork);
    (void)hipEventDestroy(h->ev_join);
    (void)hipStreamSynchronize(h->branch);
    (void)hipEventDestroy(h->ev_bfork);
    (void)hipEventDestroy(h->ev_bjoin);
    (void)hipEventDestroy(h->ev_b2join);
    if (h->branch2) (void)hipStreamSynchronize(h->branch2);
    (void)hipEventDestroy(h->ev_upd_b);
    (void)hipEventDestroy(h->ev_upd_m);
  }
  delete h;
}

int vp_pixrefer_params_changed(vp_pixrefer_t* h) {
  if (!h) return VP_ERR_ARG;
  h->params_dirty = true;
  h->vgg_dirty = true;
  h->upd_mask = 0;
  return VP_OK;
}

int vp_pixrefer_optimizer_stepped(vp_pixrefer_t* h) {
  if (!h) return VP_ERR_ARG;
  h->params_dirty = true;
  return VP_OK;
}

static int forward_impl(vp_pixrefer_t* h, const float* inputs, const float* fg_inputs, int fg_c, const float* targets, const float* masks, void* stream);

int vp_pixrefer_forward(vp_pixrefer_t* h, const float* inputs, const float* fg_inputs,
                        const float* targets, const float* masks, void* stream) {
  return forward_impl(h, inputs, fg_inputs, 6, targets, masks, stream);
}

int vp_pixrefer_forward_fg3(vp_pixrefer_t* h, const float* inputs, const float* fg_inputs3, const float* targets, void* stream) {
  if (h && h->d.training) { set_err("vp_pixrefer_forward_fg3: inference plans only (the training graph reads fg_inputs[..., 3:], pixrefer.py:297,321)"); return VP_ERR_STATE; }
  return forward_impl(h, inputs, fg_inputs3, 3, targets, nullptr, stream);
}

size_t vp_pixrefer_desc_size(void) { return sizeof(vp_pixrefer_desc); }

static int forward_impl(vp_pixrefer_t* h, const float* inputs, const float* fg_inputs, int fg_c, const float* targets, const float* masks, void* stream) {
  if (!h || !inputs || !fg_inputs || !targets) { set_err("vp_pixrefer_forward: null argument"); return VP_ERR_ARG; }
  const vp_pixrefer_desc& d = h->d;
  if (d.training && !masks) { set_err("vp_pixrefer_forward: masks required when training"); return VP_ERR_ARG; }
  hipStream_t st = (hipStream_t)stream;
  const int N = d.batch, H = d.height, bf = h->bf16;
  int rc;
  if (h->params_dirty) {
    if ((rc = run_pack(h, h->G, st))) return rc;
    if (d.training) {
      if ((rc = run_pack(h, h->D, st))) return rc;
      if (h->vgg_dirty) { if ((rc = run_pack(h, h->V, st))) return rc; h->vgg_dirty = false; }
    }
    h->params_dirty = false;
  }
  h->in_targets = targets; h->in_masks = masks;
// ... 44 lines not shown

  if (split_vgg && !vgg_real_started) { if ((rc = vgg_real_half())) return rc; vgg_real_started = true; }
  CompositeArgs ca;
  memset(&ca, 0, sizeof(ca));
  ca.y4 = h->y4; ca.targets = targets; ca.masks = masks; ca.o4 = h->o4; ca.outputs = h->outputs; ca.outputs_fg = h->outputs_fg;
  ca.din = h->din; ca.vin = h->vin; ca.partial = h->comp_partial; ca.N = N; ca.HW = H * H; ca.train = d.training;
  VP_HIP_CHECK(launch_composite_fwd(ca, bf, st));
  phase_mark(h, st, 1);
  if (!d.training) return VP_OK;

  const bool split_d = h->overlap && h->ov_on && h->dsplit_on;
  hipStream_t sd = split_d ? h->branch : st;
  const int ssd = split_d ? 2 : 0;
  if (split_d) {
    VP_HIP_CHECK(hipEventRecord(h->ev_bfork, st));
    VP_HIP_CHECK(hipStreamWaitEvent(h->branch, h->ev_bfork, 0));
  }
  for (Layer& L : h->D.l) if ((rc = run_layer_fwd(h, h->D, L, sd, nullptr, ssd))) return rc;
  const int hd = H / 8 - 2;
  GanLossArgs ga;
  memset(&ga, 0, sizeof(ga));
  ga.logits = h->logits; ga.dl_d = h->dl_d; ga.dl_g = h->dl_g; ga.predict = h->predict; ga.losses = h->losses;
  ga.M = N * hd * hd; ga.gan_weight = d.gan_weight;
  VP_HIP_CHECK(launch_gan_loss(ga, bf, sd));
  if (split_d) VP_HIP_CHECK(hipEventRecord(h->ev_bjoin, h->branch));

  Net& V = h->V;
  bool codes = split_vgg && bf && !h->store_first_raw && h->vpool_code[0] && h->vpool_code[1];
  for (Layer& L : V.l)
    if (L.scope == "conv1/conv1_2" || L.scope == "conv2/conv2_2") codes = codes && plan_can_pool(L.fwd_half);
  h->pool_codes_written = codes;
  auto vgg_half = [&](int half, hipStream_t s2) -> int {
    for (size_t i = 0; i < V.l.size(); ++i) {
      Layer& L = V.l[i];
      int rc2;
      const bool pooled = L.scope == "conv1/conv1_2" || L.scope == "conv2/conv2_2";
      const bool fuse = pooled && plan_can_pool(L.fwd_half);
      const Tens& ti = V.t[L.out];
      Tens& tp = V.t[pooled ? L.out + 1 : L.out];
      const size_t oi = (size_t)half * N * ti.H * ti.W * ti.C * h->es, op = (size_t)half * N * tp.H * tp.W * tp.C * h->es;
      const bool code = fuse && codes && half == 1;
      if ((rc2 = run_layer_fwd_half(h, V, L, half, s2, fuse ? (char*)tp.y + op : nullptr, code, code ? h->vpool_code[L.scope == "conv2/conv2_2"] : nullptr))) return rc2;
      if (pooled && !fuse) VP_HIP_CHECK(launch_maxpool_fwd((const char*)ti.y + oi, (char*)tp.y + op, N, ti.H, ti.W, ti.C, bf, s2));
    }
    return VP_OK;
  };
  if (split_vgg) {
    if ((rc = vgg_half(1, st))) return rc;
    VP_HIP_CHECK(hipStreamWaitEvent(st, h->ev_join, 0));
  } else {
    for (size_t i = 0; i < V.l.size(); ++i) {
      Layer& L = V.l[i];
      const bool pooled = L.scope == "conv1/conv1_2" || L.scope == "conv2/conv2_2";
      const bool fuse = pooled && plan_can_pool(L.fwd);
      if ((rc = run_layer_fwd(h, V, L, st, fuse ? V.t[L.out + 1].y : nullptr))) return rc;
      if (pooled && !fuse) {
        const Tens& ti = V.t[L.out];
        Tens& tp = V.t[L.out + 1];
        VP_HIP_CHECK(launch_maxpool_fwd(ti.y, tp.y, ti.N, ti.H, ti.W, ti.C, bf, st));
      }
    }
  }
  const Tens& f3 = V.t.back();
  PerceptualArgs pa;
  memset(&pa, 0, sizeof(pa));
  pa.f3 = f3.y; pa.df3 = f3.dz; pa.partial = h->perc_partial; pa.half = f3.elems() / 2; pa.l1_weight = d.l1_weight;
  VP_HIP_CHECK(launch_perceptual(pa, bf, st));

  if (split_d) VP_HIP_CHECK(hipStreamWaitEvent(st, h->ev_bjoin, 0));
  LossFinalArgs lf;
  memset(&lf, 0, sizeof(lf));
  lf.comp_partial = h->comp_partial; lf.n_comp = h->n_comp; lf.perc_partial = h->perc_partial; lf.n_perc = h->n_perc;
  lf.n_out = (double)N * H * H * 3; lf.n_feat = (double)pa.half; lf.losses = h->losses;
  lf.l1_weight = d.l1_weight; lf.gan_weight = d.gan_weight;
  VP_HIP_CHECK(launch_loss_final(lf, st));
  phase_mark(h, st, 2);
  return VP_OK;
}

static int backward_d_on(vp_pixrefer_t* h, hipStream_t st, bool side);
static int fork_d(vp_pixrefer_t* h, hipStream_t st);

static int update_range(vp_pixrefer_t* h, Net& n, float* m, float* v, float lr_t, size_t off0, size_t off1, int l0, int l1, hipStream_t s) {
  if (off1 > off0) {
    AdamArgs a;
    a.p = n.params + off0; a.g = n.grads + off0; a.m = m + off0; a.v = v + off0; a.n = off1 - off0;
    a.lr_t = lr_t; a.beta1 = h->upd.beta1; a.beta2 = h->upd.beta2; a.eps = h->upd.eps;
    VP_HIP_CHECK(launch_adam(a, s));
  }
  const size_t d0 = n.l[l0].desc0, d1 = n.l[l1].desc1;
  if (d1 > d0) VP_HIP_CHECK(launch_pack_weights(n.d_descs + d0, (int)(d1 - d0), n.params, n.packed, h->bf16, s));
  return VP_OK;
}
static int update_d(vp_pixrefer_t* h, hipStream_t s) {
  h->upd.d_done = true;
  return update_range(h, h->D, h->upd.m_d, h->upd.v_d, h->upd.lr_t_d, 0, h->D.nparams, 0, (int)h->D.l.size() - 1, s);
}

int vp_pixrefer_backward(vp_pixrefer_t* h, void* stream) {
  if (!h || !h->d.training) { set_err("vp_pixrefer_backward: needs a training plan"); return VP_ERR_STATE; }
  hipStream_t st = (hipStream_t)stream;
  if (!h->overlap || !h->ov_on) {
    int rc = vp_pixrefer_backward_d(h, stream);
    if (rc) return rc;
    return vp_pixrefer_backward_g(h, stream);
  }
  int rc;
  h->dfork_pending = h->dfork_point;
  if (h->dfork_pending == 0 && (rc = fork_d(h, st))) { h->dfork_pending = 0; return rc; }
  rc = vp_pixrefer_backward_g(h, stream);
  h->dfork_pending = 0;
  if (rc) return rc;
  VP_HIP_CHECK(hipStreamWaitEvent(st, h->ev_join, 0));
  phase_mark(h, st, 7);
  return VP_OK;
}

static int fork_d(vp_pixrefer_t* h, hipStream_t st) {
  h->dfork_pending = 0;
  VP_HIP_CHECK(hipEventRecord(h->ev_fork, st));
  VP_HIP_CHECK(hipStreamWaitEvent(h->side, h->ev_fork, 0));
  int rc = backward_d_on(h, h->side, true);
  if (rc) return rc;
  if (h->upd.active && h->dfork_point == 2 && (rc = update_d(h, h->side))) return rc;
  VP_HIP_CHECK(hipEventRecord(h->ev_join, h->side));
  return VP_OK;
}

int vp_pixrefer_backward_update(vp_pixrefer_t* h, float* m_g, float* v_g, float* m_d, float* v_d, int step_t_g, int step_t_d,
                                float lr, float beta1, float beta2, float eps, void* stream) {
  if (!h || !h->d.training) { set_err("vp_pixrefer_backward_update: needs a training plan"); return VP_ERR_STATE; }
  if (!m_g || !v_g || !m_d || !v_d || step_t_g < 1 || step_t_d < 1) { set_err("vp_pixrefer_backward_update: bad argument"); return VP_ERR_ARG; }
  auto lr_t = [&](int t) { return (float)((double)lr * sqrt(1.0 - pow((double)beta2, t)) / (1.0 - pow((double)beta1, t))); };
  h->upd.active = true; h->upd.d_done = false;
  h->upd.m_g = m_g; h->upd.v_g = v_g; h->upd.m_d = m_d; h->upd.v_d = v_d;
  h->upd.lr_t_g = lr_t(step_t_g); h->upd.lr_t_d = lr_t(step_t_d); h->upd.beta1 = beta1; h->upd.beta2 = beta2; h->upd.eps = eps;
  int rc = vp_pixrefer_backward(h, stream);
  if (!rc && !h->upd.d_done) rc = update_d(h, (hipStream_t)stream);
  h->upd.active = false;
  if (rc) return rc;
  h->params_dirty = false;
  return VP_OK;
}

int vp_pixrefer_update_bucket(vp_pixrefer_t* h, int which, int bucket, float* m, float* v, int step_t, float lr, float beta1, float beta2,
                              float eps, void* stream) {
  if (!h || !h->d.training || !m || !v || step_t < 1 || which < 0 || which > 1 || bucket < 0 || bucket > (which ? 0 : 2)) {
    set_err("vp_pixrefer_update_bucket: bad argument");
    return VP_ERR_ARG;
  }
  const float lr_t = (float)((double)lr * sqrt(1.0 - pow((double)beta2, step_t)) / (1.0 - pow((double)beta1, step_t)));
  h->upd.beta1 = beta1; h->upd.beta2 = beta2; h->upd.eps = eps;
  int rc;
  if (which == 1) {
    rc = update_range(h, h->D, m, v, lr_t, 0, h->D.nparams, 0, (int)h->D.l.size() - 1, (hipStream_t)stream);
    h->upd_mask |= 8;
  } else {
    Net& G = h->G;
    int i_md5 = -1, i_me2 = -1;
    for (int i = 0; i < (int)G.l.size(); ++i) {
      if (G.l[i].scope == "merged_decoder_5") i_md5 = i;
      if (G.l[i].scope == "merged_encoder_2") i_me2 = i;
    }
    const int l0 = bucket == 0 ? i_md5 : (bucket == 1 ? i_me2 : 0);
    const int l1 = bucket == 0 ? (int)G.l.size() - 1 : (bucket == 1 ? i_md5 - 1 : i_me2 - 1);
    const size_t off0 = G.l[l0].w_off, off1 = l1 + 1 < (int)G.l.size() ? G.l[l1 + 1].w_off : G.nparams;
    rc = update_range(h, G, m, v, lr_t, off0, off1, l0, l1, (hipStream_t)stream);
    h->upd_mask |= 1 << bucket;
  }
  if (rc) return rc;
  if (h->upd_mask == 15) { h->upd_mask = 0; h->params_dirty = false; }
  return VP_OK;
}

int vp_pixrefer_backward_d(vp_pixrefer_t* h, void* stream) {
  if (!h || !h->d.training) { set_err("vp_pixrefer_backward_d: needs a training plan"); return VP_ERR_STATE; }
  return backward_d_on(h, (hipStream_t)stream, false);
}

int vp_pixrefer_backward_d_fork(vp_pixrefer_t* h, void* stream) {
  if (!h || !h->d.training) { set_err("vp_pixrefer_backward_d_fork: needs a training plan"); return VP_ERR_STATE; }
  hipStream_t st = (hipStream_t)stream;
  h->forked = h->overlap && h->ov_on;
  if (!h->forked) return backward_d_on(h, st, false);
  h->dfork_pending = h->dfork_point;
  if (h->dfork_pending == 0) return fork_d(h, st);
  return VP_OK;
}

void* vp_pixrefer_side_stream(vp_pixrefer_t* h) { return (h && h->overlap) ? (void*)h->side : nullptr; }

int vp_pixrefer_use_streams(vp_pixrefer_t* h, int n) {
  if (!h || (n != 3 && n != 4)) { set_err("vp_pixrefer_use_streams: 3 or 4"); return VP_ERR_ARG; }
  h->use_b2 = (n == 4) && h->overlap;
  return VP_OK;
}

int vp_pixrefer_set_option(vp_pixrefer_t* h, const char* key, int value) {
  if (!h || !key) { set_err("vp_pixrefer_set_option: null argument"); return VP_ERR_ARG; }
  const std::string k(key);
  if (k == "overlap") { h->ov_on = value != 0; return VP_OK; }
  if (k == "d_backward_fork") { h->dfork_point = value < 0 ? 0 : (value > 2 ? 2 : value); return VP_OK; }
  if (k == "d_beside_vgg") { h->dsplit_on = value != 0; return VP_OK; }
  if (k == "store_first_raw") { h->store_first_raw = value != 0; return VP_OK; }
  if (k == "bwd_sums_in_epilogue") { h->bst_on = value < 0 ? 0 : (value > 2 ? 2 : value); return VP_OK; }
  if (k == "vgg_real_fork") { h->vgg_fork_layer = value < 0 ? 0 : value; return VP_OK; }
  set_err("vp_pixrefer_set_option: unknown key %s", key);
  return VP_ERR_ARG;
}

long long vp_pixrefer_counter(vp_pixrefer_t* h, const char* key) {
  if (!h || !key) return -1;
  if (std::string(key) == "bwd_sums_launches") return h->bst_count;
  if (std::string(key) == "pool_codes_written") return h->pool_codes_written ? 1 : 0;
  if (std::string(key) == "pool_bwd_fused") return h->pool_bwd_fused ? 1 : 0;
  return -1;
}

int vp_pixrefer_backward_d_join(vp_pixrefer_t* h, void* stream) {
  if (!h || !h->d.training) { set_err("vp_pixrefer_backward_d_join: needs a training plan"); return VP_ERR_STATE; }
  if (h->forked && h->dfork_pending) {
    const int rc = fork_d(h, (hipStream_t)stream);
    if (rc) return rc;
  }
  if (h->forked) VP_HIP_CHECK(hipStreamWaitEvent((hipStream_t)stream, h->ev_join, 0));
  h->forked = false;
  return VP_OK;
}

static int backward_d_on(vp_pixrefer_t* h, hipStream_t st, bool side) {
  const int N = h->d.batch;
  int rc;
  Net& D = h->D;

  for (Tens& t : D.t) { t.dz_written = false; t.bst_chunks = 0; t.cs_chunks = 0; }
  for (int i = (int)D.l.size() - 1; i >= 0; --i) {
    Layer& L = D.l[i];
    Tens& to = D.t[L.out];
    if (L.has_bn) if ((rc = run_bn_bwd(h, D, L, true, 0, 3 * N, 0, 3, st, side ? 1 : 0))) return rc;
    const bool save = L.need_bwd[0];
    if (i == 0) L.need_bwd[0] = false;
    rc = run_layer_bwd(h, D, L, to.dz, true, false, 0, 3 * N, 0, st, side ? 1 : 0);
    L.need_bwd[0] = save;
    if (rc) return rc;
  }

  return VP_OK;
}

int vp_pixrefer_backward_g(vp_pixrefer_t* h, void* stream) { return vp_pixrefer_backward_g_stage(h, -1, stream); }

int vp_pixrefer_backward_g_stages(void) { return 3; }

int vp_pixrefer_backward_g_stage(vp_pixrefer_t* h, int stage, void* stream) {
  if (!h || !h->d.training) { set_err("vp_pixrefer_backward_g: needs a training plan"); return VP_ERR_STATE; }
  if (stage > 2) { set_err("vp_pixrefer_backward_g_stage: stage must be < 3"); return VP_ERR_ARG; }
  hipStream_t st = (hipStream_t)stream;
  const vp_pixrefer_desc& d = h->d;
  const int N = d.batch, H = d.height, bf = h->bf16, es = h->es;
  int rc;
  Net &G = h->G, &D = h->D, &V = h->V;
  int i_md5 = -1, i_me2 = -1;
  for (int i = 0; i < (int)G.l.size(); ++i) {
    if (G.l[i].scope == "merged_decoder_5") i_md5 = i;
    if (G.l[i].scope == "merged_encoder_2") i_me2 = i;
  }
  const int l_hi = stage <= 0 ? (int)G.l.size() - 1 : (stage == 1 ? i_md5 - 1 : i_me2 - 1);
  const int l_lo = stage < 0 ? 0 : (stage == 0 ? i_md5 : (stage == 1 ? i_me2 : 0));
  if (stage <= 0) {
  const bool split_d = h->overlap && h->ov_on && h->dsplit_on;
  hipStream_t sd = split_d ? h->branch : st;
  const int ssd = split_d ? 2 : 0;
  if (split_d) {
    VP_HIP_CHECK(hipEventRecord(h->ev_bfork, st));
    VP_HIP_CHECK(hipStreamWaitEvent(h->branch, h->ev_bfork, 0));
  }
  for (Tens& t : D.t) { t.dz2_written = false; t.bst_chunks_g = 0; }
  for (int i = (int)D.l.size() - 1; i >= 0; --i) {
    Layer& L = D.l[i];
    Tens& to = D.t[L.out];
    if (L.has_bn) if ((rc = run_bn_bwd(h, D, L, false, 2 * N, N, 2, 1, sd, ssd, true))) return rc;
    const void* dy = (i == (int)D.l.size() - 1) ? h->dl_g : to.dz2;
    if ((rc = run_layer_bwd(h, D, L, dy, false, true, 2 * N, N, 2, sd, ssd, true))) return rc;
  }
  if (split_d) VP_HIP_CHECK(hipEventRecord(h->ev_bjoin, h->branch));
  if (h->dfork_pending == 1 && (rc = fork_d(h, st))) return rc;
  for (Tens& t : V.t) t.dz_written = false;
  h->pool_bwd_fused = false;
  h->pool_dz_stale[0] = h->pool_dz_stale[1] = false;
  for (int i = (int)V.l.size() - 1; i >= 0; --i) {
    Layer& L = V.l[i];
    Tens& to = V.t[L.out];
    Tens& ti = V.t[L.src[0]];
    IgemmArgs a = L.bwd_alt[0].a;
    set_single_src(a.x, to.dz, L.g.CoutT, nullptr, nullptr, ACT_NONE, 0);
    const int pk = L.scope == "conv2/conv2_2";
    if ((pk || L.scope == "conv1/conv1_2") && h->pool_dz_stale[pk]) {
      a.x.ptr[0] = V.t[L.out + 1].dz;
// ... 61 lines not shown
    if (wsplit && !fg) {
      VP_HIP_CHECK(hipEventRecord(h->ev_bfork, st));
      VP_HIP_CHECK(hipStreamWaitEvent(h->branch, h->ev_bfork, 0));
      forked = true;
      if ((rc = run_layer_bwd(h, G, L, to.dz, true, false, 0, N, 0, h->branch, 2, false, 1))) return rc;
      if ((rc = run_layer_bwd(h, G, L, to.dz, true, false, 0, N, 0, st, 0, false, 6))) return rc;
    } else {
      if ((rc = run_layer_bwd(h, G, L, to.dz, true, false, 0, N, 0, s2, ss))) return rc;
    }
    if (h->upd.active && (i == i_md5 || i == i_me2 || i == 0)) {
      const int l0 = i, l1 = i == i_md5 ? (int)G.l.size() - 1 : (i == i_me2 ? i_md5 - 1 : i_me2 - 1);
      const size_t off0 = G.l[l0].w_off, off1 = l1 + 1 < (int)G.l.size() ? G.l[l1 + 1].w_off : G.nparams;
      hipStream_t su = st;
      const bool on_side = h->overlap && h->ov_on && h->dfork_pending == 0 && h->dfork_point >= 0;
      if (h->overlap && h->ov_on && on_side) {
        VP_HIP_CHECK(hipEventRecord(h->ev_upd_b, h->branch));
        VP_HIP_CHECK(hipEventRecord(h->ev_upd_m, st));
        VP_HIP_CHECK(hipStreamWaitEvent(h->side, h->ev_upd_b, 0));
        VP_HIP_CHECK(hipStreamWaitEvent(h->side, h->ev_upd_m, 0));
        if (b2_used) {
          VP_HIP_CHECK(hipEventRecord(h->ev_b2join, h->branch2));
          VP_HIP_CHECK(hipStreamWaitEvent(h->side, h->ev_b2join, 0));
        }
        su = h->side;
      } else if (h->overlap && h->ov_on) {
        VP_HIP_CHECK(hipEventRecord(h->ev_bfork, st));
        VP_HIP_CHECK(hipStreamWaitEvent(h->branch, h->ev_bfork, 0));
        if (b2_used) {
          VP_HIP_CHECK(hipEventRecord(h->ev_b2join, h->branch2));
          VP_HIP_CHECK(hipStreamWaitEvent(h->branch, h->ev_b2join, 0));
        }
        su = h->branch; forked = true;
      }
      if ((rc = update_range(h, G, h->upd.m_g, h->upd.v_g, h->upd.lr_t_g, off0, off1, l0, l1, su))) return rc;
      if (h->overlap && h->ov_on && on_side) VP_HIP_CHECK(hipEventRecord(h->ev_join, h->side));
    }
  }
  if (forked) {
    if (g_phase_detail && (stage < 0 || stage == 2)) phase_mark(h, st, 60);
    VP_HIP_CHECK(hipEventRecord(h->ev_bjoin, h->branch));
    VP_HIP_CHECK(hipStreamWaitEvent(st, h->ev_bjoin, 0));
    if (b2_used) {
      VP_HIP_CHECK(hipEventRecord(h->ev_b2join, h->branch2));
      VP_HIP_CHECK(hipStreamWaitEvent(st, h->ev_b2join, 0));
    }
  }
  if (stage < 0 || stage == 2) phase_mark(h, st, 6);
  return VP_OK;
}

int vp_profile_enable(int on) { profile_enable(on); return VP_OK; }
size_t vp_profile_collect(char* json, size_t cap) { return profile_collect(json, cap); }

int vp_pixrefer_tensor(vp_pixrefer_t* h, const char* name, void** ptr, int64_t shape[4], int* dtype) {
  if (!h || !name || !ptr) return VP_ERR_ARG;
  const int N = h->d.batch, H = h->d.height;
  auto ret = [&](void* p, int64_t a, int64_t b, int64_t c, int64_t e, int dt) {
    *ptr = p;
    if (shape) { shape[0] = a; shape[1] = b; shape[2] = c; shape[3] = e; }
    if (dtype) *dtype = dt;
    return p ? VP_OK : VP_ERR_STATE;
  };
  const std::string s(name);
  const int cd = h->bf16 ? VP_BF16 : VP_F32;
  if (s == "Outputs_raw") return ret(h->outputs, N, H, H, 3, VP_F32);
  if (s == "Outputs_FG") return ret(h->outputs_fg, N, H, H, 3, VP_F32);
  if (s == "gen_out4") return ret(h->o4, N, H, H, 4, VP_F32);
  if (s == "losses") return ret(h->losses, 8, 1, 1, 1, VP_F32);
  const int hd = H / 8 - 2;
  if (s == "Predict") return ret(h->predict, 2, N, hd, hd, VP_F32);
  if (s == "logits") return ret(h->logits, 3 * N, hd, hd, 1, VP_F32);
  if (s == "d_gen_out4") return ret(h->dy4, N, H, H, 8, cd);
  if (s == "d_din") return ret(h->d_din, N, H, H, 8, cd);
  if (s == "d_vin") return ret(h->d_vin, N, H, H, 8, cd);
  const size_t c = s.find('/');
  if (c == std::string::npos) return VP_ERR_ARG;
  const std::string net = s.substr(0, c);
  std::string rest = s.substr(c + 1);
  Net* n = net == "g" ? &h->G : net == "d" ? &h->D : net == "v" ? &h->V : nullptr;
  if (!n) return VP_ERR_ARG;
  std::string field;
  const size_t k = rest.find(':');
  if (k != std::string::npos) { field = rest.substr(k + 1); rest = rest.substr(0, k); }
  for (Tens& t : n->t) {
    if (t.name != rest) continue;
    if (field.empty() && !h->store_first_raw && t.producer >= 0 && first_layer_acts_fused(h, *n, n->l[t.producer])) {
      set_err("vp_pixrefer_tensor: the raw output of %s is not stored (its kernel writes the consumers' activations); vp_pixrefer_set_option(h, \"store_first_raw\", 1) before the forward pass", s.c_str());
      return VP_ERR_STATE;
    }
    if (field.empty() && n == &h->V && h->pool_codes_written && (t.name == "conv1/conv1_2" || t.name == "conv2/conv2_2")) {
      set_err("vp_pixrefer_tensor: the full-resolution output of %s is not stored (the step keeps its 2x2 max pool and the pool's arg-max codes); vp_pixrefer_set_option(h, \"store_first_raw\", 1) before the forward pass", s.c_str());
      return VP_ERR_STATE;
    }
    if (field.empty()) return ret(t.y, t.N, t.H, t.W, t.is_f32 ? (t.name == "decoder_1" ? 4 : 1) : t.C, (t.is_f32 || t.hi) ? VP_F32 : cd);
    if (field == "dz32") return t.hi ? ret(t.dz32, t.N, t.H, t.W, t.C, VP_F32) : VP_ERR_ARG;
    if (field == "dy" && n == &h->V && (t.name == "conv1/conv1_2" || t.name == "conv2/conv2_2") && h->pool_dz_stale[t.name == "conv2/conv2_2"]) {
      const int k = t.name == "conv2/conv2_2";
      const Tens& tp = n->t[(&t - n->t.data()) + 1];
      VP_HIP_CHECK(hipDeviceSynchronize());
      VP_HIP_CHECK(launch_maxpool_bwd_code(h->vpool_code[k], tp.dz, t.dz, t.N / 2, t.H, t.W, t.C, h->bf16, nullptr));
      VP_HIP_CHECK(hipDeviceSynchronize());
      h->pool_dz_stale[k] = false;
    }
    if (field == "dy") return ret(t.dz, n == &h->V ? t.N / 2 : t.N, t.H, t.W, t.C, cd);
    if (!t.has_bn) return VP_ERR_ARG;
    if (field == "scale") return ret(t.bn.a, n->groups, t.C, 1, 1, VP_F32);
    if (field == "shift") return ret(t.bn.b, n->groups, t.C, 1, 1, VP_F32);
    if (field == "mean") return ret(t.bn.mu, n->groups, t.C, 1, 1, VP_F32);
    if (field == "rstd") return ret(t.bn.rstd, n->groups, t.C, 1, 1, VP_F32);
    return VP_ERR_ARG;
  }
  return VP_ERR_ARG;
}

int vp_pixrefer_fetch(vp_pixrefer_t* h, int what, void* dst, void* stream) {
  if (!h || !dst || what < 0 || what > 3) { set_err("vp_pixrefer_fetch: bad argument"); return VP_ERR_ARG; }
  FetchArgs f;
  memset(&f, 0, sizeof(f));
  f.raw3 = h->outputs; f.fg3 = h->outputs_fg; f.o4 = h->o4; f.dst = dst;
  f.npix = (size_t)h->d.batch * h->d.height * h->d.height;
  f.mode = what;
  if (what == 3 && h->d.training) {
    VP_HIP_CHECK(hipMemcpyAsync(dst, h->outputs_fg, f.npix * 3 * sizeof(float), hipMemcpyDeviceToDevice, (hipStream_t)stream));
    return VP_OK;
  }
  VP_HIP_CHECK(launch_fetch(f, (hipStream_t)stream));
  return VP_OK;
}

int vp_grad_pack_bf16(const float* src, void* dst_bf16, size_t n, void* stream) {
  if (!src || !dst_bf16 || n < 1 || ((uintptr_t)src & 31) || ((uintptr_t)dst_bf16 & 15)) { set_err("vp_grad_pack_bf16: bad argument"); return VP_ERR_ARG; }
  VP_HIP_CHECK(launch_grad_pack_bf16(src, dst_bf16, n, (hipStream_t)stream));
  return VP_OK;
}
int vp_grad_unpack_bf16(const void* src_bf16, float* dst, size_t n, float scale, void* stream) {
  if (!src_bf16 || !dst || n < 1 || ((uintptr_t)dst & 31) || ((uintptr_t)src_bf16 & 15)) { set_err("vp_grad_unpack_bf16: bad argument"); return VP_ERR_ARG; }
  VP_HIP_CHECK(launch_grad_unpack_bf16(src_bf16, dst, n, scale, (hipStream_t)stream));
  return VP_OK;
}

int vp_adam_tf(float* params, const float* grads, float* m, float* v, size_t n, int step_t,
               float lr, float beta1, float beta2, float eps, void* stream) {
  if (!params || !grads || !m || !v || step_t < 1) { set_err("vp_adam_tf: bad argument"); return VP_ERR_ARG; }
  AdamArgs a;
  a.p = params; a.g = grads; a.m = m; a.v = v; a.n = n;
  a.lr_t = (float)((double)lr * sqrt(1.0 - pow((double)beta2, step_t)) / (1.0 - pow((double)beta1, step_t)));
  a.beta1 = beta1; a.beta2 = beta2; a.eps = eps;
  VP_HIP_CHECK(launch_adam(a, (hipStream_t)stream));
  return VP_OK;
}

}
```

voicepuppet_amd/csrc/pointwise.hip:

```cpp
#include "pointwise_args.h"
#include "vp_common.h"

namespace vp {

template <int NV>
__device__ __forceinline__ void block_sum(double (&v)[NV], double* sm ) {
  const int lane = threadIdx.x & 63, wave = threadIdx.x >> 6, nw = blockDim.x >> 6;
#pragma unroll
  for (int i = 0; i < NV; ++i) v[i] = wave_sum(v[i]);
  __syncthreads();
  if (lane == 0)
#pragma unroll
    for (int i = 0; i < NV; ++i) sm[i * 16 + wave] = v[i];
  __syncthreads();
  if (threadIdx.x == 0)
#pragma unroll
    for (int i = 0; i < NV; ++i) {
      double s = 0;
      for (int w = 0; w < nw; ++w) s += sm[i * 16 + w];
      v[i] = s;
    }
}

template <typename T>
__global__ __launch_bounds__(256) void pack_weights_kernel(const PackDesc* __restrict__ descs, const float* __restrict__ master, T* __restrict__ packed) {
  constexpr int E = Elem<T>::E;
  const PackDesc& d = descs[blockIdx.y];
  const int npiece = d.Kpad / E;
  const int total = d.nclass * d.rows_pad * npiece;
  T* dst = packed + d.dst_off;
  const float* src = master + d.src_off;
  const bool row_fast = d.s_row == 1;
  if (row_fast && d.kc == 4 * E) {
    const int nchk = d.Kpad / d.kc;
    const int total4 = d.nclass * d.rows_pad * nchk;
    for (int i = blockIdx.x * 256 + threadIdx.x; i < total4; i += gridDim.x * 256) {
      const int row = i % d.rows_pad, t = i / d.rows_pad, chk = t % nchk, cls = t / nchk;
      const int prow = d.perm ? perm_row(row) : row;
      T* o = dst + (((size_t)cls * nchk + chk) * d.rows_pad + prow) * d.kc;
#pragma unroll
      for (int j = 0; j < 4; ++j) {
        const int k0 = chk * d.kc + j * E;
        const int tap = k0 / d.C, c0 = k0 - tap * d.C;
        float v[E];
#pragma unroll
        for (int e = 0; e < E; ++e) v[e] = 0.f;
        if (row < d.rows_real && tap < d.ntaps) {
          const float* p = src + (size_t)d.kh[cls][tap] * d.s_kh + (size_t)d.kw[cls][tap] * d.s_kw + (size_t)row * d.s_row + (size_t)c0 * d.s_ch;
#pragma unroll
          for (int e = 0; e < E; ++e) if (c0 + e < d.C_real) v[e] = p[(size_t)e * d.s_ch];
        }
        if (d.kswap && (j & 1)) {
#pragma unroll
          for (int e = 0; e < E / 2; ++e) { const float tmp = v[e]; v[e] = v[e + E / 2]; v[e + E / 2] = tmp; }
        }
        reinterpret_cast<uint4*>(o)[j] = Elem<T>::pack(v);
      }
    }
    return;
  }
  for (int i = blockIdx.x * 256 + threadIdx.x; i < total; i += gridDim.x * 256) {
    int row, piece, cls;
    if (row_fast) { row = i % d.rows_pad; const int t = i / d.rows_pad; piece = t % npiece; cls = t / npiece; }
    else { piece = i % npiece; const int t = i / npiece; row = t % d.rows_pad; cls = t / d.rows_pad; }
    const int k0 = piece * E;
    const int tap = k0 / d.C, c0 = k0 - tap * d.C;
    float v[E];
#pragma unroll
    for (int e = 0; e < E; ++e) v[e] = 0.f;
    if (row < d.rows_real && tap < d.ntaps) {
      const float* p = src + (size_t)d.kh[cls][tap] * d.s_kh + (size_t)d.kw[cls][tap] * d.s_kw + (size_t)row * d.s_row + (size_t)c0 * d.s_ch;
#pragma unroll
      for (int e = 0; e < E; ++e) if (c0 + e < d.C_real) v[e] = p[(size_t)e * d.s_ch];
    }
    const int prow = d.perm ? perm_row(row) : row;
    T* o = dst + (((size_t)cls * (d.Kpad / d.kc) + k0 / d.kc) * d.rows_pad + prow) * d.kc + k0 % d.kc;
    if (d.kswap && (piece & 1)) {
#pragma unroll
      for (int e = 0; e < E / 2; ++e) { const float tmp = v[e]; v[e] = v[e + E / 2]; v[e + E / 2] = tmp; }
    }
    *reinterpret_cast<uint4*>(o) = Elem<T>::pack(v);
  }
// ... 648 lines not shown
    Elem<T>::unpack(*reinterpret_cast<const uint4*>(p + (size_t)W * C + C), v);
#pragma unroll
    for (int e = 0; e < E; ++e) m[e] = fmaxf(m[e], v[e]);
    *reinterpret_cast<uint4*>(y + i * E) = Elem<T>::pack(m);
  }
}

template <typename T>
__global__ __launch_bounds__(256) void maxpool_bwd_kernel(const T* __restrict__ x, const T* __restrict__ dy, T* __restrict__ dx, int B, int H, int W, int C) {
  constexpr int E = Elem<T>::E;
  const int ncg = C / E, Ho = H / 2, Wo = W / 2;
  const size_t total = (size_t)B * Ho * Wo * ncg;
  for (size_t i = (size_t)blockIdx.x * 256 + threadIdx.x; i < total; i += (size_t)gridDim.x * 256) {
    const int cg = (int)(i % ncg);
    size_t t = i / ncg;
    const int ow = (int)(t % Wo); t /= Wo;
    const int oh = (int)(t % Ho);
    const int n = (int)(t / Ho);
    const size_t base = (((size_t)n * H + 2 * oh) * W + 2 * ow) * C + cg * E;
    const size_t offs[4] = {0, (size_t)C, (size_t)W * C, (size_t)W * C + C};
    float v[4][E], g[E];
#pragma unroll
    for (int k = 0; k < 4; ++k) Elem<T>::unpack(*reinterpret_cast<const uint4*>(x + base + offs[k]), v[k]);
    Elem<T>::unpack(*reinterpret_cast<const uint4*>(dy + i * E), g);
    float o[4][E];
#pragma unroll
    for (int e = 0; e < E; ++e) {
      int best = 0;
      float m = v[0][e];
#pragma unroll
      for (int k = 1; k < 4; ++k) if (v[k][e] > m) { m = v[k][e]; best = k; }
#pragma unroll
      for (int k = 0; k < 4; ++k) o[k][e] = (k == best && m > 0.f) ? g[e] : 0.f;
    }
#pragma unroll
    for (int k = 0; k < 4; ++k) *reinterpret_cast<uint4*>(dx + base + offs[k]) = Elem<T>::pack(o[k]);
  }
}

template <typename T>
__global__ __launch_bounds__(256) void maxpool_bwd_code_kernel(const unsigned char* __restrict__ code, const T* __restrict__ dy, T* __restrict__ dx, int B, int H, int W, int C) {
  constexpr int E = Elem<T>::E;
  const int ncg = C / E, Ho = H / 2, Wo = W / 2;
  const size_t total = (size_t)B * Ho * Wo * ncg;
  for (size_t i = (size_t)blockIdx.x * 256 + threadIdx.x; i < total; i += (size_t)gridDim.x * 256) {
    const int cg = (int)(i % ncg);
    size_t t = i / ncg;
    const int ow = (int)(t % Wo); t /= Wo;
    const int oh = (int)(t % Ho);
    const int n = (int)(t / Ho);
    const size_t base = (((size_t)n * H + 2 * oh) * W + 2 * ow) * C + cg * E;
    const size_t offs[4] = {0, (size_t)C, (size_t)W * C, (size_t)W * C + C};
    unsigned cw[2];
    if constexpr (E == 8) { const uint2 c2 = *reinterpret_cast<const uint2*>(code + i * E); cw[0] = c2.x; cw[1] = c2.y; }
    else { cw[0] = *reinterpret_cast<const unsigned*>(code + i * E); cw[1] = 0; }
    float g[E];
    Elem<T>::unpack(*reinterpret_cast<const uint4*>(dy + i * E), g);
    float o[4][E];
#pragma unroll
    for (int e = 0; e < E; ++e) {
      const unsigned c = (cw[e >> 2] >> (8 * (e & 3))) & 0xffu;
#pragma unroll
      for (int k = 0; k < 4; ++k) o[k][e] = c == (unsigned)(k + 1) ? g[e] : 0.f;
    }
#pragma unroll
    for (int k = 0; k < 4; ++k) *reinterpret_cast<uint4*>(dx + base + offs[k]) = Elem<T>::pack(o[k]);
  }
}

template <typename T>
__global__ __launch_bounds__(256) void relu_bwd_kernel(const T* __restrict__ y, T* __restrict__ d, size_t nvec) {
  constexpr int E = Elem<T>::E;
  for (size_t i = (size_t)blockIdx.x * 256 + threadIdx.x; i < nvec; i += (size_t)gridDim.x * 256) {
    float fy[E], fd[E];
    Elem<T>::unpack(reinterpret_cast<const uint4*>(y)[i], fy);
    Elem<T>::unpack(reinterpret_cast<const uint4*>(d)[i], fd);
#pragma unroll
    for (int e = 0; e < E; ++e) fd[e] = fy[e] > 0.f ? fd[e] : 0.f;
    reinterpret_cast<uint4*>(d)[i] = Elem<T>::pack(fd);
  }
}

__global__ __launch_bounds__(256) void adam_tf_kernel(const AdamArgs a) {
  for (size_t i = (size_t)blockIdx.x * 256 + threadIdx.x; i < a.n; i += (size_t)gridDim.x * 256) {
    const float g = a.g[i];
    const float m = a.beta1 * a.m[i] + (1.f - a.beta1) * g;
    const float v = a.beta2 * a.v[i] + (1.f - a.beta2) * g * g;
    a.m[i] = m; a.v[i] = v;
    a.p[i] -= a.lr_t * m / (sqrtf(v) + a.eps);
  }
}

__global__ __launch_bounds__(256) void grad_pack_bf16_kernel(const float* __restrict__ src, bf16* __restrict__ dst, size_t n8, size_t n) {
  for (size_t i = (size_t)blockIdx.x * 256 + threadIdx.x; i < n8; i += (size_t)gridDim.x * 256) {
    const float4 a = reinterpret_cast<const float4*>(src)[2 * i], b = reinterpret_cast<const float4*>(src)[2 * i + 1];
    const float f[8] = {a.x, a.y, a.z, a.w, b.x, b.y, b.z, b.w};
    reinterpret_cast<uint4*>(dst)[i] = Elem<bf16>::pack(f);
  }
  if (blockIdx.x == 0 && threadIdx.x < (int)(n - n8 * 8)) Elem<bf16>::st(dst + n8 * 8 + threadIdx.x, src[n8 * 8 + threadIdx.x]);
}

__global__ __launch_bounds__(256) void grad_unpack_bf16_kernel(const bf16* __restrict__ src, float* __restrict__ dst, size_t n8, size_t n, float scale) {
  for (size_t i = (size_t)blockIdx.x * 256 + threadIdx.x; i < n8; i += (size_t)gridDim.x * 256) {
    float f[8];
    Elem<bf16>::unpack(reinterpret_cast<const uint4*>(src)[i], f);
    reinterpret_cast<float4*>(dst)[2 * i] = make_float4(f[0] * scale, f[1] * scale, f[2] * scale, f[3] * scale);
    reinterpret_cast<float4*>(dst)[2 * i + 1] = make_float4(f[4] * scale, f[5] * scale, f[6] * scale, f[7] * scale);
  }
  if (blockIdx.x == 0 && threadIdx.x < (int)(n - n8 * 8)) dst[n8 * 8 + threadIdx.x] = Elem<bf16>::ld(src + n8 * 8 + threadIdx.x) * scale;
}

static inline int nblocks(size_t work, int cap = 2048) {
  size_t b = (work + 255) / 256;
  if (b < 1) b = 1;
  return (int)(b > (size_t)cap ? cap : b);
}

#define VP_DISPATCH(is_bf16, KERNEL, grid, block, stream, ...)                         \
  do {                                                                                 \
    if (is_bf16) hipLaunchKernelGGL((KERNEL<bf16>), grid, block, 0, stream, __VA_ARGS__); \
    else hipLaunchKernelGGL((KERNEL<float>), grid, block, 0, stream, __VA_ARGS__);       \
  } while (0)

__global__ __launch_bounds__(256) void fetch_kernel(const FetchArgs a) {
  for (size_t p = (size_t)blockIdx.x * 256 + threadIdx.x; p < a.npix; p += (size_t)gridDim.x * 256) {
    float v[3];
    if (a.mode == 0 || a.mode == 1) {
#pragma unroll
      for (int c = 0; c < 3; ++c) v[c] = __fmul_rn(__fadd_rn(a.raw3[p * 3 + c], 1.f), 0.5f);
    } else {
      const float al = __fmul_rn(__fadd_rn(a.o4[p * 4 + 3], 1.f), 0.5f);
#pragma unroll
      for (int c = 0; c < 3; ++c)
        v[c] = a.mode == 2 ? al : __fmul_rn(__fadd_rn(__fsub_rn(__fadd_rn(a.fg3[p * 3 + c], al), 1.f), 1.f), 0.5f);
    }
    if (a.mode == 1) {
      unsigned char* o = reinterpret_cast<unsigned char*>(a.dst) + p * 3;
#pragma unroll
      for (int c = 0; c < 3; ++c) o[c] = (unsigned char)(int)__fmul_rn(fminf(fmaxf(v[c], 0.f), 1.f), 255.f);
    } else {
      float* o = reinterpret_cast<float*>(a.dst) + p * 3;
#pragma unroll
      for (int c = 0; c < 3; ++c) o[c] = v[c];
    }
  }
}

hipError_t launch_fetch(const FetchArgs& a, hipStream_t st) {
  hipLaunchKernelGGL(fetch_kernel, dim3(nblocks(a.npix, 4096)), dim3(256), 0, st, a);
  return hipGetLastError();
}

hipError_t launch_pack_weights(const PackDesc* d_descs, int ndesc, const float* master, void* packed, int is_bf16, hipStream_t st) {
  dim3 grid(512, ndesc);
  if (is_bf16) hipLaunchKernelGGL((pack_weights_kernel<bf16>), grid, dim3(256), 0, st, d_descs, master, (bf16*)packed);
  else hipLaunchKernelGGL((pack_weights_kernel<float>), grid, dim3(256), 0, st, d_descs, master, (float*)packed);
  return hipGetLastError();
}

hipError_t launch_pack_weights_one(const PackDesc& d, const float* master, void* packed, int is_bf16, hipStream_t st) {
  if (is_bf16) hipLaunchKernelGGL((pack_weights_one_kernel<bf16>), dim3(512), dim3(256), 0, st, d, master, (bf16*)packed);
  else hipLaunchKernelGGL((pack_weights_one_kernel<float>), dim3(512), dim3(256), 0, st, d, master, (float*)packed);
  return hipGetLastError();
}

int bn_nchunk(int Pg, int C, int G, int is_bf16) {
  const int E = is_bf16 ? 8 : 4;
  const int nprow = 256 / (C / E);
  int n = (Pg + nprow * 8 - 1) / (nprow * 8);
  const int cap = 1024 / G;
  if (n > cap) n = cap;
  return n < 1 ? 1 : n;
// ... 87 lines not shown

hipError_t launch_tap_spread(const TapArgs& a, int is_bf16, hipStream_t st) {
  VP_DISPATCH(is_bf16, tap_spread_kernel, dim3((unsigned)(((size_t)a.N * a.Hin * a.Win + 255) / 256)), dim3(256), st, a);
  return hipGetLastError();
}

hipError_t launch_pack_inputs(const PackInputsArgs& a, int is_bf16, hipStream_t st) {
  VP_DISPATCH(is_bf16, pack_inputs_kernel, dim3(nblocks((size_t)a.N * a.HW)), dim3(256), st, a);
  return hipGetLastError();
}

hipError_t launch_frame_pack(const FramePackArgs& a, hipStream_t st) {
  hipLaunchKernelGGL(frame_pack_kernel, dim3(nblocks((size_t)a.N * a.S * a.S * 2)), dim3(256), 0, st, a);
  return hipGetLastError();
}

int composite_nblocks(int N, int HW) { return nblocks((size_t)N * HW, 1024); }

hipError_t launch_composite_fwd(const CompositeArgs& a, int is_bf16, hipStream_t st) {
  VP_DISPATCH(is_bf16, composite_fwd_kernel, dim3(composite_nblocks(a.N, a.HW)), dim3(256), st, a);
  return hipGetLastError();
}

hipError_t launch_composite_bwd(const CompositeArgs& a, int is_bf16, hipStream_t st) {
  VP_DISPATCH(is_bf16, composite_bwd_kernel, dim3(nblocks((size_t)a.N * a.HW)), dim3(256), st, a);
  return hipGetLastError();
}

hipError_t launch_gan_loss(const GanLossArgs& a, int is_bf16, hipStream_t st) {
  VP_DISPATCH(is_bf16, gan_loss_kernel, dim3(1), dim3(1024), st, a);
  return hipGetLastError();
}

int perceptual_nblocks(size_t half, int is_bf16) { return nblocks(half / (is_bf16 ? 8 : 4), 1024); }

hipError_t launch_perceptual(const PerceptualArgs& a, int is_bf16, hipStream_t st) {
  VP_DISPATCH(is_bf16, perceptual_kernel, dim3(perceptual_nblocks(a.half, is_bf16)), dim3(256), st, a);
  return hipGetLastError();
}

hipError_t launch_loss_final(const LossFinalArgs& a, hipStream_t st) {
  hipLaunchKernelGGL(loss_final_kernel, dim3(1), dim3(256), 0, st, a);
  return hipGetLastError();
}

hipError_t launch_maxpool_fwd(const void* x, void* y, int B, int H, int W, int C, int is_bf16, hipStream_t st) {
  const size_t work = (size_t)B * (H / 2) * (W / 2) * (C / (is_bf16 ? 8 : 4));
  if (is_bf16) hipLaunchKernelGGL((maxpool_fwd_kernel<bf16>), dim3(nblocks(work)), dim3(256), 0, st, (const bf16*)x, (bf16*)y, B, H, W, C);
  else hipLaunchKernelGGL((maxpool_fwd_kernel<float>), dim3(nblocks(work)), dim3(256), 0, st, (const float*)x, (float*)y, B, H, W, C);
  return hipGetLastError();
}

hipError_t launch_maxpool_bwd(const void* x, const void* dy, void* dx, int B, int H, int W, int C, int is_bf16, hipStream_t st) {
  const size_t work = (size_t)B * (H / 2) * (W / 2) * (C / (is_bf16 ? 8 : 4));
  if (is_bf16) hipLaunchKernelGGL((maxpool_bwd_kernel<bf16>), dim3(nblocks(work)), dim3(256), 0, st, (const bf16*)x, (const bf16*)dy, (bf16*)dx, B, H, W, C);
  else hipLaunchKernelGGL((maxpool_bwd_kernel<float>), dim3(nblocks(work)), dim3(256), 0, st, (const float*)x, (const float*)dy, (float*)dx, B, H, W, C);
  return hipGetLastError();
}

hipError_t launch_maxpool_bwd_code(const void* code, const void* dy, void* dx, int B, int H, int W, int C, int is_bf16, hipStream_t st) {
  const size_t work = (size_t)B * (H / 2) * (W / 2) * (C / (is_bf16 ? 8 : 4));
  if (is_bf16) hipLaunchKernelGGL((maxpool_bwd_code_kernel<bf16>), dim3(nblocks(work)), dim3(256), 0, st, (const unsigned char*)code, (const bf16*)dy, (bf16*)dx, B, H, W, C);
  else hipLaunchKernelGGL((maxpool_bwd_code_kernel<float>), dim3(nblocks(work)), dim3(256), 0, st, (const unsigned char*)code, (const float*)dy, (float*)dx, B, H, W, C);
  return hipGetLastError();
}

hipError_t launch_relu_bwd(const void* y, void* d, size_t n, int is_bf16, hipStream_t st) {
  const size_t nvec = n / (is_bf16 ? 8 : 4);
  if (is_bf16) hipLaunchKernelGGL((relu_bwd_kernel<bf16>), dim3(nblocks(nvec)), dim3(256), 0, st, (const bf16*)y, (bf16*)d, nvec);
  else hipLaunchKernelGGL((relu_bwd_kernel<float>), dim3(nblocks(nvec)), dim3(256), 0, st, (const float*)y, (float*)d, nvec);
  return hipGetLastError();
}

hipError_t launch_grad_pack_bf16(const float* src, void* dst, size_t n, hipStream_t st) {
  hipLaunchKernelGGL(grad_pack_bf16_kernel, dim3(nblocks(n / 8 + 1, 4096)), dim3(256), 0, st, src, (bf16*)dst, n / 8, n);
  return hipGetLastError();
}

hipError_t launch_grad_unpack_bf16(const void* src, float* dst, size_t n, float scale, hipStream_t st) {
  hipLaunchKernelGGL(grad_unpack_bf16_kernel, dim3(nblocks(n / 8 + 1, 4096)), dim3(256), 0, st, (const bf16*)src, dst, n / 8, n, scale);
  return hipGetLastError();
}

hipError_t launch_adam(const AdamArgs& a, hipStream_t st) {
  hipLaunchKernelGGL(adam_tf_kernel, dim3(nblocks(a.n, 4096)), dim3(256), 0, st, a);
  return hipGetLastError();
}

}
```

voicepuppet_amd/csrc/pointwise_args.h:

```cpp
#pragma once
#include <stddef.h>
#include <stdint.h>

namespace vp {

struct PackDesc {
  size_t src_off;
  size_t dst_off;
  int nclass, rows_real, rows_pad, ntaps, C, C_real, Kpad;
  int kc;
  int perm;
  int kswap;
  int s_kh, s_kw, s_row, s_ch;
  int8_t kh[4][16];
  int8_t kw[4][16];
};

struct FetchArgs {
  const float* raw3;
  const float* fg3;
  const float* o4;
  void* dst;
  size_t npix;
  int mode;
// ... 21 lines not shown
  float* dbias_zero;
  int raw;
};

struct PackInputsArgs {
  const float* inputs;
  const float* fg_inputs;
  void* gin;
  void* gfg;
  void* din;
  void* vin;
  int N, HW, train;
  int fg_c;
};

struct FramePackArgs {
  const unsigned char* ex;
  const unsigned char* cur;
  const int* crops;
  float* inputs;
  float* fg_inputs;
  float* targets;
  float* masks;
  int N, S;
};

struct CompositeArgs {
  const float* y4;
  const float* targets;
  const float* masks;
  float* o4;
  float* outputs;
  float* outputs_fg;
  void* din;
  void* vin;
  double* partial;
  int N, HW, train;
  const void* d_din;
  const void* d_vin;
  void* dy4;
  float l1_weight;
};

struct GanLossArgs {
  const float* logits;
  void* dl_d;
  void* dl_g;
  float* predict;
  float* losses;
  int M;
  float gan_weight;
};

struct PerceptualArgs {
  const void* f3;
  void* df3;
  double* partial;
  size_t half;
  float l1_weight;
};

struct LossFinalArgs {
  const double* comp_partial; int n_comp;
  const double* perc_partial; int n_perc;
  double n_out;
  double n_feat;
  float* losses;
  float l1_weight, gan_weight;
};

struct TapArgs {
  const float* S;
  const float* bias;
  float* y;
  const void* dy;
  void* dyS;
  int N, Hin, Win, Hout, Wout, ks, pad, ld_dy;
};

struct AdamArgs {
  float* p; const float* g; float* m; float* v;
  size_t n;
  float lr_t, beta1, beta2, eps;
};

}
```

Measured before the change: 4577 frames/s.

## Fuse Adam update with packed-weight repack and vectorize Adam kernel

Adds an optional kernel that applies the TF-Adam update on 64x64 weight tiles and writes the updated weights straight into the packed GEMM layout from shared memory. This removes the separate weight-pack pass that re-reads the parameters after each optimizer step. A host-side planner builds tiles and views and checks that coverage is exact, with fallbacks for layers that cannot be tiled. The plain Adam kernel is also changed to use float4 accesses with an aligned head and tail. The fused path sits behind a knob that defaults to off.

```diff
diff --git a/include/vp_hip.h b/include/vp_hip.h
--- a/include/vp_hip.h
+++ b/include/vp_hip.h
@@ -67,6 +67,9 @@
 int vp_pixrefer_use_streams(vp_pixrefer_t* h, int n);
 int vp_pixrefer_set_option(vp_pixrefer_t* h, const char* key, int value);
 long long vp_pixrefer_counter(vp_pixrefer_t* h, const char* key);
+int vp_pixrefer_adam_pack_info(const vp_pixrefer_desc* d, int which, long long* out);
+int vp_pixrefer_adam_pack_descs(const vp_pixrefer_desc* d, int which, void* descs_out, int* fused_out);
+int vp_pixrefer_adam_pack_image(const vp_pixrefer_desc* d, int which, int desc_index, int* out, size_t n_out);
 int vp_pixrefer_fetch(vp_pixrefer_t* h, int what, void* dst, void* stream);
 int vp_pixrefer_backward_g_stages(void);
 int vp_pixrefer_backward_g_stage(vp_pixrefer_t* h, int stage, void* stream);
diff --git a/voicepuppet_amd/_lib.py b/voicepuppet_amd/_lib.py
--- a/voicepuppet_amd/_lib.py
+++ b/voicepuppet_amd/_lib.py
@@ -105,6 +105,9 @@
     "vp_pixrefer_set_option": (ctypes.c_int, [_P, ctypes.c_char_p, ctypes.c_int]),
     "vp_pixrefer_fetch": (ctypes.c_int, [_P, ctypes.c_int, _P, _P]),
     "vp_pixrefer_counter": (ctypes.c_longlong, [_P, ctypes.c_char_p]),
+    "vp_pixrefer_adam_pack_info": (ctypes.c_int, [ctypes.POINTER(PixReferDesc), ctypes.c_int, ctypes.POINTER(ctypes.c_longlong)]),
+    "vp_pixrefer_adam_pack_descs": (ctypes.c_int, [ctypes.POINTER(PixReferDesc), ctypes.c_int, _P, _P]),
+    "vp_pixrefer_adam_pack_image": (ctypes.c_int, [ctypes.POINTER(PixReferDesc), ctypes.c_int, ctypes.c_int, _P, ctypes.c_size_t]),
     "vp_crc32c": (ctypes.c_uint, [_P, ctypes.c_size_t, ctypes.c_uint]),
     "vp_pixrefer_phase_ms": (ctypes.c_int, [_P, ctypes.POINTER(ctypes.c_float), ctypes.c_int]),
     "vp_grad_pack_bf16": (ctypes.c_int, [_P, _P, ctypes.c_size_t, _P]),
diff --git a/voicepuppet_amd/csrc/adam_pack.hip b/voicepuppet_amd/csrc/adam_pack.hip
--- /dev/null
+++ b/voicepuppet_amd/csrc/adam_pack.hip
@@ -0,0 +1,81 @@
+#include "adam_pack_args.h"
+#include "launch.h"
+#include "vp_common.h"
+
+namespace vp {
+
+constexpr int AP_LD = AP_TILE + 1;
+
+template <typename T>
+__global__ __launch_bounds__(256) void adam_pack_kernel(const AdamPackArgs a) {
+  constexpr int E = Elem<T>::E;
+  const ApTile t = a.tiles[blockIdx.x];
+  const int tid = threadIdx.x;
+  if (t.n) {
+    for (unsigned i = tid; i < t.n; i += 256) {
+      const size_t o = (size_t)t.off + i;
+      float p = a.p[o], m = a.m[o], v = a.v[o];
+      adam_tf_elem(p, a.g[o], m, v, a.lr_t, a.beta1, a.beta2, a.eps);
+      a.m[o] = m; a.v[o] = v; a.p[o] = p;
+    }
+    return;
+  }
+  __shared__ float tile[AP_TILE * AP_LD];
+  {
+    const int col = (tid & 15) * 4, row = tid >> 4;
+    float4 p[4], g[4], m[4], v[4];
+#pragma unroll
+    for (int i = 0; i < 4; ++i) {
+      const size_t o = (size_t)t.off + (size_t)(row + 16 * i) * t.B + col;
+      p[i] = *reinterpret_cast<const float4*>(a.p + o);
+      g[i] = *reinterpret_cast<const float4*>(a.g + o);
+      m[i] = *reinterpret_cast<const float4*>(a.m + o);
+      v[i] = *reinterpret_cast<const float4*>(a.v + o);
+    }
+#pragma unroll
+    for (int i = 0; i < 4; ++i) {
+      const size_t o = (size_t)t.off + (size_t)(row + 16 * i) * t.B + col;
+      adam_tf_elem(p[i].x, g[i].x, m[i].x, v[i].x, a.lr_t, a.beta1, a.beta2, a.eps);
+      adam_tf_elem(p[i].y, g[i].y, m[i].y, v[i].y, a.lr_t, a.beta1, a.beta2, a.eps);
+      adam_tf_elem(p[i].z, g[i].z, m[i].z, v[i].z, a.lr_t, a.beta1, a.beta2, a.eps);
+      adam_tf_elem(p[i].w, g[i].w, m[i].w, v[i].w, a.lr_t, a.beta1, a.beta2, a.eps);
+      *reinterpret_cast<float4*>(a.m + o) = m[i];
+      *reinterpret_cast<float4*>(a.v + o) = v[i];
+      *reinterpret_cast<float4*>(a.p + o) = p[i];
+      float* l = tile + (row + 16 * i) * AP_LD + col;
+      l[0] = p[i].x; l[1] = p[i].y; l[2] = p[i].z; l[3] = p[i].w;
+    }
+  }
+  __syncthreads();
+  T* const packed = reinterpret_cast<T*>(a.packed);
+  for (int vi = 0; vi < t.nview; ++vi) {
+    const PackDesc& d = a.descs[t.view0 + vi];
+    const ApView& w = a.views[t.view0 + vi];
+    size_t dst, cstride;
+    if (!ap_view_base(d, w, t, &dst, &cstride)) continue;
+    const int perm = d.perm, kswap = d.kswap, rowa = w.row_is_a;
+#pragma unroll
+    for (int q = tid; q < AP_TILE * AP_TILE / E; q += 256) {
+      const ApPiece pc = ap_piece(q, E, perm, cstride);
+      const float* s = rowa ? tile + pc.r * AP_LD + pc.c : tile + pc.c * AP_LD + pc.r;
+      const int ss = rowa ? 1 : AP_LD;
+      float f[E];
+#pragma unroll
+      for (int e = 0; e < E; ++e) f[e] = s[e * ss];
+      if (kswap && pc.odd) {
+#pragma unroll
+        for (int e = 0; e < E / 2; ++e) { const float tmp = f[e]; f[e] = f[e + E / 2]; f[e + E / 2] = tmp; }
+      }
+      *reinterpret_cast<uint4*>(packed + dst + pc.dst) = Elem<T>::pack(f);
+    }
+  }
+}
+
+hipError_t launch_adam_pack(const AdamPackArgs& a, int is_bf16, hipStream_t st) {
+  if (a.ntiles < 1) return hipSuccess;
+  if (is_bf16) hipLaunchKernelGGL((adam_pack_kernel<bf16>), dim3(a.ntiles), dim3(256), 0, st, a);
+  else hipLaunchKernelGGL((adam_pack_kernel<float>), dim3(a.ntiles), dim3(256), 0, st, a);
+  return hipGetLastError();
+}
+
+}
diff --git a/voicepuppet_amd/csrc/adam_pack_args.h b/voicepuppet_amd/csrc/adam_pack_args.h
--- /dev/null
+++ b/voicepuppet_amd/csrc/adam_pack_args.h
@@ -0,0 +1,73 @@
+#pragma once
+#include <hip/hip_runtime.h>
+#include <stddef.h>
+#include <stdint.h>
+
+#include "pointwise_args.h"
+
+namespace vp {
+
+constexpr int AP_TILE = 64;
+
+struct ApView {
+  int row_is_a;
+  int row0;
+  uint8_t inv[16];
+};
+
+struct ApTile {
+  unsigned off;
+  unsigned n;
+  int view0, nview;
+  int B;
+  int tap, a0, b0;
+};
+
+__host__ __device__ inline int ap_unperm_row(int p) {
+  return (p & ~63) | (((p >> 5) & 1) << 5) | (((p >> 2) & 3) << 3) | (((p >> 4) & 1) << 2) | (p & 3);
+}
+
+__host__ __device__ inline bool ap_view_base(const PackDesc& d, const ApView& w, const ApTile& t, size_t* dst, size_t* chunk_stride) {
+  const unsigned ct = w.inv[t.tap];
+  if (ct == 0xffu) return false;
+  const int rb = (w.row_is_a ? t.a0 : t.b0) - w.row0;
+  if (rb < 0 || rb >= d.rows_real) return false;
+  const int cb = w.row_is_a ? t.b0 : t.a0;
+  const int cls = (int)(ct >> 4), tp = (int)(ct & 15u);
+  *dst = d.dst_off + (((size_t)cls * (d.Kpad / d.kc) + (size_t)((tp * d.C + cb) / d.kc)) * d.rows_pad + rb) * d.kc;
+  *chunk_stride = (size_t)d.rows_pad * d.kc;
+  return true;
+}
+
+struct ApPiece { size_t dst; int r, c, odd; };
+__host__ __device__ inline ApPiece ap_piece(int q, int E, int perm, size_t chunk_stride) {
+  const int chl = q >> 8, prow = (q >> 2) & 63, j = q & 3;
+  ApPiece p;
+  p.dst = (size_t)chl * chunk_stride + (size_t)prow * (4 * E) + (size_t)j * E;
+  p.r = perm ? ap_unperm_row(prow) : prow;
+  p.c = chl * 4 * E + j * E;
+  p.odd = j & 1;
+  return p;
+}
+
+struct AdamPackArgs {
+  const ApTile* tiles;
+  const ApView* views;
+  const PackDesc* descs;
+  float* p; const float* g; float* m; float* v;
+  void* packed;
+  int ntiles;
+  float lr_t, beta1, beta2, eps;
+};
+
+#if defined(__HIPCC__)
+__device__ __forceinline__ void adam_tf_elem(float& p, float g, float& m, float& v, float lr_t, float beta1, float beta2, float eps) {
+#pragma clang fp contract(off)
+  const float m1 = beta1 * m + (1.f - beta1) * g;
+  const float v1 = beta2 * v + (1.f - beta2) * g * g;
+  m = m1; v = v1;
+  p -= lr_t * m1 / (sqrtf(v1) + eps);
+}
+#endif
+
+}
diff --git a/voicepuppet_amd/csrc/conv_ops.h b/voicepuppet_amd/csrc/conv_ops.h
--- a/voicepuppet_amd/csrc/conv_ops.h
+++ b/voicepuppet_amd/csrc/conv_ops.h
@@ -116,6 +116,7 @@
 inline int& patch4_knob() { static int v = 1; return v; }
 inline int& c64_knob() { static int v = 1; return v; }
 inline int& pool_bwd_fused_knob() { static int v = 1; return v; }
+inline int& adam_pack_knob() { static int v = 0; return v; }
 inline int& cout1_knob() { static int v = 256; return v; }
 inline int& wgrad1_rows_knob() { static int v = 512; return v; }
 inline int& dc64_knob() { static int v = 1; return v; }
diff --git a/voicepuppet_amd/csrc/launch.h b/voicepuppet_amd/csrc/launch.h
--- a/voicepuppet_amd/csrc/launch.h
+++ b/voicepuppet_amd/csrc/launch.h
@@ -82,6 +82,8 @@
 hipError_t launch_maxpool_bwd_code(const void* code, const void* dy, void* dx, int B, int H, int W, int C, int is_bf16, hipStream_t st);
 hipError_t launch_relu_bwd(const void* y, void* d, size_t n, int is_bf16, hipStream_t st);
 hipError_t launch_adam(const AdamArgs& a, hipStream_t st);
+struct AdamPackArgs;
+hipError_t launch_adam_pack(const AdamPackArgs& a, int is_bf16, hipStream_t st);
 hipError_t launch_fetch(const FetchArgs& a, hipStream_t st);
 hipError_t launch_grad_pack_bf16(const float* src, void* dst, size_t n, hipStream_t st);
 hipError_t launch_grad_unpack_bf16(const void* src, float* dst, size_t n, float scale, hipStream_t st);
diff --git a/voicepuppet_amd/csrc/ops_api.hip b/voicepuppet_amd/csrc/ops_api.hip
--- a/voicepuppet_amd/csrc/ops_api.hip
+++ b/voicepuppet_amd/csrc/ops_api.hip
@@ -66,6 +66,7 @@
   if (k == "c64") { c64_knob() = value; return VP_OK; }
   if (k == "dc64") { dc64_knob() = value; return VP_OK; }
   if (k == "pool_bwd_fused") { pool_bwd_fused_knob() = value < 0 || value > 4 ? 1 : value; return VP_OK; }
+  if (k == "adam_pack_fused") { adam_pack_knob() = value != 0; return VP_OK; }
   if (k == "cout1_wgrad_rows" && value > 0) { wgrad1_rows_knob() = value; return VP_OK; }
   if (k == "cout1_bwd") { cout1_knob() = value < 0 ? 256 : value; return VP_OK; }
   if (k == "s2c64") { s2c64_knob() = value; return VP_OK; }
diff --git a/voicepuppet_amd/csrc/plan_pixrefer.hip b/voicepuppet_amd/csrc/plan_pixrefer.hip
--- a/voicepuppet_amd/csrc/plan_pixrefer.hip
+++ b/voicepuppet_amd/csrc/plan_pixrefer.hip
@@ -7,6 +7,7 @@
 #include <utility>
 #include <vector>
 
+#include "adam_pack_args.h"
 #include "conv_ops.h"
 #include "errors.h"
 #include "launch.h"
@@ -89,6 +90,9 @@
   bool has_fwd_half = false;
   WgradPlan wg;
   size_t desc0 = 0, desc1 = 0;
+  size_t ap_tile0 = 0, ap_tile1 = 0, ap_rest0 = 0, ap_rest1 = 0;
+  bool ap_fused = false;
+  bool ap_ran = false;
   bool tapgemm = false;
   bool fwd_stats = false;
   float* tap_S = nullptr;
@@ -112,6 +116,13 @@
   size_t packed_elems = 0;
   std::vector<PackDesc> descs;
   PackDesc* d_descs = nullptr;
+  std::vector<ApTile> ap_tiles;
+  std::vector<ApView> ap_views;
+  std::vector<PackDesc> ap_rest;
+  ApTile* d_ap_tiles = nullptr;
+  ApView* d_ap_views = nullptr;
+  PackDesc* d_ap_rest = nullptr;
+  size_t ap_fused_elems = 0, ap_weight_elems = 0;
   unsigned* sp_cnt = nullptr;
   size_t sp_cnt_n = 0;
 };
@@ -454,6 +465,176 @@
   }
 }
 
+static void ap_dims(const Layer& L, int* A, int* B) {
+  if (L.g.kind == 0) { *A = L.g.Cin_real; *B = L.g.Cout; } else { *A = L.g.Cout; *B = L.g.Cin_real; }
+}
+
+static bool ap_make_view(const Layer& L, const PackDesc& d, int E, ApView* w) {
+  int A, B;
+  ap_dims(L, &A, &B);
+  const int ks = L.g.ks;
+  memset(w, 0, sizeof(*w));
+  if (d.kc != 4 * E || d.C != d.C_real || d.C % AP_TILE || d.rows_real % AP_TILE || d.rows_real > d.rows_pad || d.Kpad % d.kc ||
+      d.Kpad < d.ntaps * d.C || d.nclass < 1 || d.nclass > 4 || d.ntaps < 1 || d.ntaps > 16 || d.dst_off % d.kc)
+    return false;
+  if (d.s_kh != ks * A * B || d.s_kw != A * B) return false;
+  int len;
+  if (d.s_row == 1 && d.s_ch == B) { w->row_is_a = 0; len = B; if (d.C != A) return false; }
+  else if (d.s_row == B && d.s_ch == 1) { w->row_is_a = 1; len = A; if (d.C != B) return false; }
+  else return false;
+  if (d.src_off < L.w_off) return false;
+  const size_t rel = d.src_off - L.w_off;
+  if (rel % (size_t)d.s_row || rel / (size_t)d.s_row >= (size_t)len) return false;
+  w->row0 = (int)(rel / (size_t)d.s_row);
+  if (w->row0 % AP_TILE || w->row0 + d.rows_real > len) return false;
+  memset(w->inv, 0xff, sizeof(w->inv));
+  for (int cls = 0; cls < d.nclass; ++cls)
+    for (int t = 0; t < d.ntaps; ++t) {
+      const int kh = d.kh[cls][t], kw = d.kw[cls][t];
+      if (kh < 0 || kh >= ks || kw < 0 || kw >= ks) return false;
+      uint8_t& e = w->inv[kh * ks + kw];
+      if (e != 0xff) return false;
+      e = (uint8_t)(cls << 4 | t);
+    }
+  return true;
+}
+
+static void plan_adam_pack(Net& n, int bf16, bool on) {
+  const int E = bf16 ? 8 : 4;
+  n.ap_tiles.clear(); n.ap_views.clear(); n.ap_rest.clear();
+  n.ap_fused_elems = n.ap_weight_elems = 0;
+  n.ap_views.resize(n.descs.size());
+  for (ApView& w : n.ap_views) { memset(&w, 0, sizeof(w)); memset(w.inv, 0xff, sizeof(w.inv)); }
+  auto plain = [&](size_t o0, size_t o1) {
+    for (size_t o = o0; o < o1; o += 1024) {
+      ApTile t;
+      memset(&t, 0, sizeof(t));
+      t.off = (unsigned)o; t.n = (unsigned)(o1 - o < 1024 ? o1 - o : 1024);
+      n.ap_tiles.push_back(t);
+    }
+  };
+  for (size_t li = 0; li < n.l.size(); ++li) {
+    Layer& L = n.l[li];
+    int A, B;
+    ap_dims(L, &A, &B);
+    const int taps = L.g.ks * L.g.ks;
+    const size_t wn = (size_t)taps * A * B, end = li + 1 < n.l.size() ? n.l[li + 1].w_off : n.nparams;
+    n.ap_weight_elems += wn;
+    L.ap_tile0 = n.ap_tiles.size(); L.ap_rest0 = n.ap_rest.size();
+    L.ap_fused = false; L.ap_ran = false;
+    bool ok = on && !L.tapgemm && taps <= 16 && A % AP_TILE == 0 && B % AP_TILE == 0 && L.w_off % 4 == 0 && L.b_off == L.w_off + wn &&
+              n.nparams < ((size_t)1 << 31) && L.desc1 > L.desc0;
+    for (size_t i = L.desc0; i < L.desc1 && ok; ++i) ok = ap_make_view(L, n.descs[i], E, &n.ap_views[i]);
+    if (on) {
+      if (ok) {
+        L.ap_fused = true;
+        n.ap_fused_elems += wn;
+        for (int tap = 0; tap < taps; ++tap)
+          for (int a0 = 0; a0 < A; a0 += AP_TILE)
+            for (int b0 = 0; b0 < B; b0 += AP_TILE) {
+              ApTile t;
+              memset(&t, 0, sizeof(t));
+              t.off = (unsigned)(L.w_off + ((size_t)tap * A + a0) * B + b0);
+              t.view0 = (int)L.desc0; t.nview = (int)(L.desc1 - L.desc0);
+              t.B = B; t.tap = tap; t.a0 = a0; t.b0 = b0;
+              n.ap_tiles.push_back(t);
+            }
+        plain(L.w_off + wn, end);
+      } else {
+        plain(L.w_off, end);
+        for (size_t i = L.desc0; i < L.desc1; ++i) n.ap_rest.push_back(n.descs[i]);
+      }
+    }
+    L.ap_tile1 = n.ap_tiles.size(); L.ap_rest1 = n.ap_rest.size();
+  }
+}
+
+static void ap_replay(const Net& n, int bf16, int* master, long long di, int* img) {
+  const int E = bf16 ? 8 : 4;
+  for (const Layer& L : n.l) {
+    const bool mine = di >= 0 && (size_t)di >= L.desc0 && (size_t)di < L.desc1;
+    if (!master && !mine) continue;
+    for (size_t ti = L.ap_tile0; ti < L.ap_tile1; ++ti) {
+      const ApTile& t = n.ap_tiles[ti];
+      if (t.n) { if (master) for (unsigned i = 0; i < t.n; ++i) master[t.off + i]++; continue; }
+      if (master)
+        for (int r = 0; r < AP_TILE; ++r)
+          for (int c = 0; c < AP_TILE; ++c) master[(size_t)t.off + (size_t)r * t.B + c]++;
+      if (!mine || di < t.view0 || di >= t.view0 + t.nview) continue;
+      const PackDesc& d = n.descs[di];
+      const ApView& w = n.ap_views[di];
+      size_t dst, cs;
+      if (!ap_view_base(d, w, t, &dst, &cs)) continue;
+      for (int q = 0; q < AP_TILE * AP_TILE / E; ++q) {
+        const ApPiece pc = ap_piece(q, E, d.perm, cs);
+        for (int e = 0; e < E; ++e) {
+          const int es = (d.kswap && pc.odd) ? (e + E / 2) % E : e;
+          const size_t src = (size_t)t.off + (w.row_is_a ? (size_t)pc.r * t.B + pc.c + es : (size_t)(pc.c + es) * t.B + pc.r);
+          int& o = img[dst + pc.dst + e - d.dst_off];
+          o = o == -1 ? (int)src : -2;
+        }
+      }
+    }
+  }
+}
+
+static std::string ap_check(const Net& n, int bf16) {
+  if (n.ap_tiles.empty()) return "";
+  char msg[256];
+  const int E = bf16 ? 8 : 4;
+  std::vector<int> master(n.nparams, 0);
+  ap_replay(n, bf16, master.data(), -1, nullptr);
+  for (size_t i = 0; i < n.nparams; ++i)
+    if (master[i] != 1) { snprintf(msg, sizeof(msg), "adam_pack: arena element %zu is updated %d times", i, master[i]); return msg; }
+  std::vector<int> img;
+  for (const Layer& L : n.l) {
+    for (size_t di = L.desc0; di < L.desc1; ++di) {
+      const PackDesc& d = n.descs[di];
+      const size_t pe = (size_t)d.nclass * d.rows_pad * d.Kpad;
+      if (d.dst_off + pe > n.packed_elems) { snprintf(msg, sizeof(msg), "adam_pack: %s view %zu outside the packed arena", L.scope.c_str(), di); return msg; }
+      img.assign(pe, -1);
+      for (size_t ti = L.ap_tile0; ti < L.ap_tile1; ++ti) {
+        const ApTile& t = n.ap_tiles[ti];
+        size_t dst, cs;
+        if (t.n || !ap_view_base(d, n.ap_views[di], t, &dst, &cs)) continue;
+        if (dst < d.dst_off || dst - d.dst_off + (size_t)(AP_TILE / d.kc - 1) * cs + (size_t)AP_TILE * d.kc > pe) {
+          snprintf(msg, sizeof(msg), "adam_pack: %s view %zu: a tile lands outside the view's block", L.scope.c_str(), di);
+          return msg;
+        }
+      }
+      ap_replay(n, bf16, nullptr, (long long)di, img.data());
+      size_t written = 0, real = 0;
+      for (size_t e = 0; e < pe; ++e) {
+        if (img[e] == -2) { snprintf(msg, sizeof(msg), "adam_pack: %s view %zu: packed element %zu written twice", L.scope.c_str(), di, e); return msg; }
+        if (img[e] >= 0) ++written;
+      }
+      if (L.ap_fused) {
+        const int nchk = d.Kpad / d.kc;
+        for (int cls = 0; cls < d.nclass; ++cls)
+          for (int tap = 0; tap < d.ntaps; ++tap)
+            for (int row = 0; row < d.rows_real; ++row) {
+              const size_t sb = d.src_off + (size_t)d.kh[cls][tap] * d.s_kh + (size_t)d.kw[cls][tap] * d.s_kw + (size_t)row * d.s_row;
+              const int prow = d.perm ? perm_row(row) : row;
+              for (int c = 0; c < d.C_real; ++c) {
+                const int k = tap * d.C + c;
+                int kk = k % d.kc;
+                if (d.kswap && ((kk / E) & 1)) kk = (kk / E) * E + ((kk % E) + E / 2) % E;
+                const size_t e = (((size_t)cls * nchk + k / d.kc) * d.rows_pad + prow) * d.kc + kk;
+                ++real;
+                if (img[e] != (int)(sb + (size_t)c * d.s_ch)) {
+                  snprintf(msg, sizeof(msg), "adam_pack: %s view %zu (class %d tap %d row %d c %d): source %d, expected %zu", L.scope.c_str(), di, cls, tap,
+                           row, c, img[e], sb + (size_t)c * d.s_ch);
+                  return msg;
+                }
+              }
+            }
+      }
+      if (written != real) { snprintf(msg, sizeof(msg), "adam_pack: %s view %zu: %zu elements written, %zu real", L.scope.c_str(), di, written, real); return msg; }
+    }
+  }
+  return "";
+}
+
 static void carve_net(Net& n, Arena& ar, int es, bool training) {
   for (Tens& t : n.t) {
     if (t.name == "decoder_1" || t.name == "layer_5") {
@@ -479,6 +660,11 @@
   }
   n.packed = (char*)ar.alloc(n.packed_elems * es);
   n.d_descs = (PackDesc*)ar.alloc(n.descs.size() * sizeof(PackDesc));
+  if (!n.ap_tiles.empty()) {
+    n.d_ap_tiles = (ApTile*)ar.alloc(n.ap_tiles.size() * sizeof(ApTile));
+    n.d_ap_views = (ApView*)ar.alloc(n.ap_views.size() * sizeof(ApView));
+    n.d_ap_rest = (PackDesc*)ar.alloc((n.ap_rest.size() + 1) * sizeof(PackDesc));
+  }
   n.sp_cnt = (unsigned*)ar.alloc((n.sp_cnt_n + 1) * sizeof(unsigned));
   {
     unsigned* c = n.sp_cnt;
@@ -567,6 +753,8 @@
   if (d->training) {
     build_discriminator(h->D, d->batch, d->height, d->ndf);
     plan_net(h->D, h->bf16, true, true, d->batch, &smax);
+    plan_adam_pack(h->G, h->bf16, adam_pack_knob() != 0);
+    plan_adam_pack(h->D, h->bf16, adam_pack_knob() != 0);
     build_vgg(h->V, d->batch, d->height);
     for (Layer& L : h->V.l) L.g.N = 2 * d->batch;
     plan_net(h->V, h->bf16, true, false, d->batch, &smax, true);
@@ -1151,6 +1339,13 @@
       if (p.dst_off + pe > n->packed_elems) fail("pack block [%zu, +%zu) outside the %zu-element packed arena", p.dst_off, pe, n->packed_elems);
       if (p.src_off >= n->nparams) fail("pack source %zu outside the %zu-float parameter arena", p.src_off, n->nparams);
     }
+    if (!n->ap_tiles.empty()) {
+      region_of(n->d_ap_tiles, n->ap_tiles.size() * sizeof(ApTile), "adam_pack tiles");
+      region_of(n->d_ap_views, n->ap_views.size() * sizeof(ApView), "adam_pack views");
+      region_of(n->d_ap_rest, (n->ap_rest.size() + 1) * sizeof(PackDesc), "adam_pack leftover descriptors");
+      const std::string m = ap_check(*n, h->bf16);
+      if (!m.empty()) fail("%s", m.c_str());
+    }
     size_t pend = 0;
     for (const ParamInfo& p : n->manifest) {
       size_t cnt = 1;
@@ -1203,6 +1398,49 @@
     region_of(h->scratch2, h->scratch_bytes, "scratch2"); region_of(h->scratch3, h->scratch_bytes, "scratch3");
     region_of(h->scratch4, h->scratch_bytes, "scratch4"); region_of(h->bn_partial4, (size_t)1024 * 2 * 512 * 8, "bn_partial4");
     region_of(h->bn_partial2, (size_t)1024 * 2 * 512 * 8, "bn_partial2"); region_of(h->bn_partial3, (size_t)1024 * 2 * 512 * 8, "bn_partial3");
+  }
+  delete h;
+  return rc;
+}
+
+static vp_pixrefer* ap_host_plan(const vp_pixrefer_desc* d, int which, Net** n) {
+  if (!valid_desc(d) || !d->training || which < 0 || which > 1) { set_err("vp_pixrefer_adam_pack_*: needs a training descriptor and net 0 / 1"); return nullptr; }
+  vp_pixrefer* h = new vp_pixrefer{};
+  init_handle(h, d);
+  *n = which ? &h->D : &h->G;
+  return h;
+}
+int vp_pixrefer_adam_pack_info(const vp_pixrefer_desc* d, int which, long long* out) {
+  Net* n;
+  vp_pixrefer* h = ap_host_plan(d, which, &n);
+  if (!h || !out) { delete h; return VP_ERR_ARG; }
+  out[0] = (long long)n->nparams; out[1] = (long long)n->packed_elems; out[2] = (long long)n->descs.size(); out[3] = (long long)n->ap_weight_elems;
+  out[4] = (long long)n->ap_fused_elems; out[5] = (long long)n->ap_tiles.size(); out[6] = (long long)sizeof(PackDesc); out[7] = (long long)n->ap_rest.size();
+  delete h;
+  return VP_OK;
+}
+int vp_pixrefer_adam_pack_descs(const vp_pixrefer_desc* d, int which, void* descs_out, int* fused_out) {
+  Net* n;
+  vp_pixrefer* h = ap_host_plan(d, which, &n);
+  if (!h || !descs_out || !fused_out) { delete h; return VP_ERR_ARG; }
+  memcpy(descs_out, n->descs.data(), n->descs.size() * sizeof(PackDesc));
+  for (const Layer& L : n->l)
+    for (size_t i = L.desc0; i < L.desc1; ++i) fused_out[i] = L.ap_fused ? 1 : 0;
+  delete h;
+  return VP_OK;
+}
+int vp_pixrefer_adam_pack_image(const vp_pixrefer_desc* d, int which, int di, int* out, size_t n_out) {
+  Net* n;
+  vp_pixrefer* h = ap_host_plan(d, which, &n);
+  if (!h || !out) { delete h; return VP_ERR_ARG; }
+  int rc = VP_OK;
+  if (di < 0) {
+    if (n_out != n->nparams) { set_err("vp_pixrefer_adam_pack_image: %zu counts for a %zu-float arena", n_out, n->nparams); rc = VP_ERR_ARG; }
+    else { memset(out, 0, n_out * sizeof(int)); ap_replay(*n, h->bf16, out, -1, nullptr); }
+  } else {
+    const size_t pe = (size_t)di < n->descs.size() ? (size_t)n->descs[di].nclass * n->descs[di].rows_pad * n->descs[di].Kpad : 0;
+    if (!pe || n_out != pe) { set_err("vp_pixrefer_adam_pack_image: descriptor %d has %zu packed elements, got room for %zu", di, pe, n_out); rc = VP_ERR_ARG; }
+    else { for (size_t i = 0; i < pe; ++i) out[i] = -1; ap_replay(*n, h->bf16, nullptr, di, out); }
   }
   delete h;
   return rc;
@@ -1263,6 +1501,11 @@
     if (n->descs.empty()) continue;
     VP_HIP_CHECK(hipMemcpyAsync(n->d_descs, n->descs.data(), n->descs.size() * sizeof(PackDesc), hipMemcpyHostToDevice, st));
     VP_HIP_CHECK(hipMemsetAsync(n->sp_cnt, 0, (n->sp_cnt_n + 1) * sizeof(unsigned), st));
+    if (!n->ap_tiles.empty()) {
+      VP_HIP_CHECK(hipMemcpyAsync(n->d_ap_tiles, n->ap_tiles.data(), n->ap_tiles.size() * sizeof(ApTile), hipMemcpyHostToDevice, st));
+      VP_HIP_CHECK(hipMemcpyAsync(n->d_ap_views, n->ap_views.data(), n->ap_views.size() * sizeof(ApView), hipMemcpyHostToDevice, st));
+      if (!n->ap_rest.empty()) VP_HIP_CHECK(hipMemcpyAsync(n->d_ap_rest, n->ap_rest.data(), n->ap_rest.size() * sizeof(PackDesc), hipMemcpyHostToDevice, st));
+    }
   }
   VP_HIP_CHECK(hipStreamSynchronize(st));
   h->overlap = false; h->forked = false;
@@ -1473,6 +1716,21 @@
 static int fork_d(vp_pixrefer_t* h, hipStream_t st);
 
 static int update_range(vp_pixrefer_t* h, Net& n, float* m, float* v, float lr_t, size_t off0, size_t off1, int l0, int l1, hipStream_t s) {
+  const size_t lay_end = l1 + 1 < (int)n.l.size() ? n.l[l1 + 1].w_off : n.nparams;
+  const bool al16 = (((uintptr_t)n.params | (uintptr_t)n.grads | (uintptr_t)m | (uintptr_t)v) & 15) == 0;
+  const bool fused = !n.ap_tiles.empty() && al16 && off0 == n.l[l0].w_off && off1 == lay_end;
+  for (int i = l0; i <= l1; ++i) n.l[i].ap_ran = fused && n.l[i].ap_fused;
+  if (fused) {
+    AdamPackArgs a;
+    a.tiles = n.d_ap_tiles + n.l[l0].ap_tile0; a.ntiles = (int)(n.l[l1].ap_tile1 - n.l[l0].ap_tile0);
+    a.views = n.d_ap_views; a.descs = n.d_descs;
+    a.p = n.params; a.g = n.grads; a.m = m; a.v = v; a.packed = n.packed;
+    a.lr_t = lr_t; a.beta1 = h->upd.beta1; a.beta2 = h->upd.beta2; a.eps = h->upd.eps;
+    VP_HIP_CHECK(launch_adam_pack(a, h->bf16, s));
+    const size_t r0 = n.l[l0].ap_rest0, r1 = n.l[l1].ap_rest1;
+    if (r1 > r0) VP_HIP_CHECK(launch_pack_weights(n.d_ap_rest + r0, (int)(r1 - r0), n.params, n.packed, h->bf16, s));
+    return VP_OK;
+  }
   if (off1 > off0) {
     AdamArgs a;
     a.p = n.params + off0; a.g = n.grads + off0; a.m = m + off0; a.v = v + off0; a.n = off1 - off0;
@@ -1605,6 +1863,13 @@
   if (std::string(key) == "bwd_sums_launches") return h->bst_count;
   if (std::string(key) == "pool_codes_written") return h->pool_codes_written ? 1 : 0;
   if (std::string(key) == "pool_bwd_fused") return h->pool_bwd_fused ? 1 : 0;
+  if (std::string(key) == "adam_pack_fused_elems") {
+    long long e = 0;
+    for (const Net* n : {&h->G, &h->D})
+      for (const Layer& L : n->l)
+        if (L.ap_ran) { int A, B; ap_dims(L, &A, &B); e += (long long)L.g.ks * L.g.ks * A * B; }
+    return e;
+  }
   return -1;
 }
 
@@ -1832,6 +2097,7 @@
   std::string field;
   const size_t k = rest.find(':');
   if (k != std::string::npos) { field = rest.substr(k + 1); rest = rest.substr(0, k); }
+  if (rest.empty() && field == "packed") return ret(n->packed, (int64_t)n->packed_elems, 1, 1, 1, cd);
   for (Tens& t : n->t) {
     if (t.name != rest) continue;
     if (field.empty() && !h->store_first_raw && t.producer >= 0 && first_layer_acts_fused(h, *n, n->l[t.producer])) {
diff --git a/voicepuppet_amd/csrc/pointwise.hip b/voicepuppet_amd/csrc/pointwise.hip
--- a/voicepuppet_amd/csrc/pointwise.hip
+++ b/voicepuppet_amd/csrc/pointwise.hip
@@ -1,3 +1,4 @@
+#include "adam_pack_args.h"
 #include "pointwise_args.h"
 #include "vp_common.h"
 
@@ -812,12 +813,35 @@
 }
 
 __global__ __launch_bounds__(256) void adam_tf_kernel(const AdamArgs a) {
-  for (size_t i = (size_t)blockIdx.x * 256 + threadIdx.x; i < a.n; i += (size_t)gridDim.x * 256) {
-    const float g = a.g[i];
-    const float m = a.beta1 * a.m[i] + (1.f - a.beta1) * g;
-    const float v = a.beta2 * a.v[i] + (1.f - a.beta2) * g * g;
-    a.m[i] = m; a.v[i] = v;
-    a.p[i] -= a.lr_t * m / (sqrtf(v) + a.eps);
+  if (a.head < 0) {
+    for (size_t i = (size_t)blockIdx.x * 256 + threadIdx.x; i < a.n; i += (size_t)gridDim.x * 256) {
+      float p = a.p[i], m = a.m[i], v = a.v[i];
+      adam_tf_elem(p, a.g[i], m, v, a.lr_t, a.beta1, a.beta2, a.eps);
+      a.m[i] = m; a.v[i] = v; a.p[i] = p;
+    }
+    return;
+  }
+  const size_t head = (size_t)a.head, n4 = (a.n - head) / 4, tail0 = head + 4 * n4;
+  float4* const p4 = reinterpret_cast<float4*>(a.p + head);
+  const float4* const g4 = reinterpret_cast<const float4*>(a.g + head);
+  float4* const m4 = reinterpret_cast<float4*>(a.m + head);
+  float4* const v4 = reinterpret_cast<float4*>(a.v + head);
+  for (size_t i = (size_t)blockIdx.x * 256 + threadIdx.x; i < n4; i += (size_t)gridDim.x * 256) {
+    float4 p = p4[i], m = m4[i], v = v4[i];
+    const float4 g = g4[i];
+    adam_tf_elem(p.x, g.x, m.x, v.x, a.lr_t, a.beta1, a.beta2, a.eps);
+    adam_tf_elem(p.y, g.y, m.y, v.y, a.lr_t, a.beta1, a.beta2, a.eps);
+    adam_tf_elem(p.z, g.z, m.z, v.z, a.lr_t, a.beta1, a.beta2, a.eps);
+    adam_tf_elem(p.w, g.w, m.w, v.w, a.lr_t, a.beta1, a.beta2, a.eps);
+    m4[i] = m; v4[i] = v; p4[i] = p;
+  }
+  if (blockIdx.x == 0 && threadIdx.x < 8) {
+    const size_t i = threadIdx.x < 4 ? threadIdx.x : tail0 + (threadIdx.x - 4);
+    if (threadIdx.x < 4 ? i < head : i < a.n) {
+      float p = a.p[i], m = a.m[i], v = a.v[i];
+      adam_tf_elem(p, a.g[i], m, v, a.lr_t, a.beta1, a.beta2, a.eps);
+      a.m[i] = m; a.v[i] = v; a.p[i] = p;
+    }
   }
 }
 
@@ -1071,7 +1095,12 @@
   return hipGetLastError();
 }
 
-hipError_t launch_adam(const AdamArgs& a, hipStream_t st) {
+hipError_t launch_adam(const AdamArgs& a0, hipStream_t st) {
+  AdamArgs a = a0;
+  const uintptr_t mis = (uintptr_t)a.p & 15;
+  const bool same = ((uintptr_t)a.g & 15) == mis && ((uintptr_t)a.m & 15) == mis && ((uintptr_t)a.v & 15) == mis && mis % 4 == 0;
+  a.head = same ? (int)(((16 - mis) & 15) / 4) : -1;
+  if (a.head >= 0 && (size_t)a.head > a.n) a.head = (int)a.n;
   hipLaunchKernelGGL(adam_tf_kernel, dim3(nblocks(a.n, 4096)), dim3(256), 0, st, a);
   return hipGetLastError();
 }
diff --git a/voicepuppet_amd/csrc/pointwise_args.h b/voicepuppet_amd/csrc/pointwise_args.h
--- a/voicepuppet_amd/csrc/pointwise_args.h
+++ b/voicepuppet_amd/csrc/pointwise_args.h
@@ -127,6 +127,7 @@
   float* p; const float* g; float* m; float* v;
   size_t n;
   float lr_t, beta1, beta2, eps;
+  int head;
 };
 
 }
```

Result: no change. 4539 frames/s (-0.8%).
